# lgen-sudo/EgoM2P

Measured on NVIDIA B200. Metric: ego-b mod4 train nominal tokens/sec (whole job), higher is better.
Workload: dtype bf16

## Files before the change

egom2p_b200/csrc/attn_bwd.cu:

```cuda
#include "attn_common.cuh"

namespace egom2p {

constexpr int kBwdMathWarps = 8;
constexpr int kBwdThreads = 32 * (kBwdMathWarps + 7);
constexpr int kDrainWarp0 = kBwdMathWarps, kBwdTmaWarp = kBwdMathWarps + 4, kBwdMmaWarp = kBwdMathWarps + 5,
              kBwdMmaWarpB = kBwdMathWarps + 6;
constexpr int kBwdStages = 3;
constexpr int kBwdMetaBytes = 5 * kT * 4;
constexpr int kMaxQBlocks = 1024;

struct BwdParams {
  int B, H, Mq, Nk, S;
  RangeMeta meta;
  const float* lse2;
  const float* ndelta;
  float scale_log2;
  uint16_t* dK;
  uint16_t* dV;
  int64_t lddk, lddv;
  int tma_out;
};
struct BwdSmem {
  static constexpr int kTile = kT * 128;
  static constexpr int kK = 0, kV = kK + kTile, kQ = kV + kTile, kDO = kQ + kBwdStages * kTile,
                       kDS = kDO + kBwdStages * kTile,
                       kBox = kDS + 2 * kTile,
                       kMeta = kBox + 8 * 4096, kList = kMeta + kBwdStages * kBwdMetaBytes,
                       kBar = kList + kMaxQBlocks * 2, kTotal = kBar + 256 + 1024;
};
static_assert(BwdSmem::kTotal <= 232448, "attention backward exceeds the 227 KB shared memory of one CTA");


#ifdef EGOM2P_TRACE
__device__ long long g_trace[16 * 64];
#define TRACE(slot, idx)                                                                          \
  do {                                                                                            \
    if (blockIdx.x == 0 && blockIdx.y == 0 && blockIdx.z == gridDim.z - 1 && (idx) < 64 && (threadIdx.x & 31) == 0) \
      g_trace[(slot) * 64 + (idx)] = clock64();                                                   \
  } while (0)
#else
#define TRACE(slot, idx) do {} while (0)
#endif

__device__ __forceinline__ void tmem_st32(uint32_t taddr, const uint32_t (&r)[32]) {
  asm volatile(
      "tcgen05.st.sync.aligned.32x32b.x32.b32 [%0], "
      "{%1, %2, %3, %4, %5, %6, %7, %8, %9, %10, %11, %12, %13, %14, %15, %16, "
      "%17, %18, %19, %20, %21, %22, %23, %24, %25, %26, %27, %28, %29, %30, %31, %32};"
      ::"r"(taddr), "r"(r[0]), "r"(r[1]), "r"(r[2]), "r"(r[3]), "r"(r[4]), "r"(r[5]), "r"(r[6]), "r"(r[7]), "r"(r[8]),
        "r"(r[9]), "r"(r[10]), "r"(r[11]), "r"(r[12]), "r"(r[13]), "r"(r[14]), "r"(r[15]), "r"(r[16]), "r"(r[17]),
        "r"(r[18]), "r"(r[19]), "r"(r[20]), "r"(r[21]), "r"(r[22]), "r"(r[23]), "r"(r[24]), "r"(r[25]), "r"(r[26]),
        "r"(r[27]), "r"(r[28]), "r"(r[29]), "r"(r[30]), "r"(r[31])
      : "memory");
}
__device__ __forceinline__ void tmem_st16(uint32_t taddr, const uint32_t (&r)[16]) {
  asm volatile(
      "tcgen05.st.sync.aligned.32x32b.x16.b32 [%0], "
      "{%1, %2, %3, %4, %5, %6, %7, %8, %9, %10, %11, %12, %13, %14, %15, %16};"
      ::"r"(taddr), "r"(r[0]), "r"(r[1]), "r"(r[2]), "r"(r[3]), "r"(r[4]), "r"(r[5]), "r"(r[6]), "r"(r[7]), "r"(r[8]),
        "r"(r[9]), "r"(r[10]), "r"(r[11]), "r"(r[12]), "r"(r[13]), "r"(r[14]), "r"(r[15])
      : "memory");
}
__device__ __forceinline__ void tmem_st_wait() { asm volatile("tcgen05.wait::st.sync.aligned;" ::: "memory"); }
__device__ __forceinline__ float4 lds_f4(const void* p) {
  float4 v;
  asm volatile("ld.shared.v4.f32 {%0, %1, %2, %3}, [%4];" : "=f"(v.x), "=f"(v.y), "=f"(v.z), "=f"(v.w) : "r"(smem_u32(p)));
  return v;
}

__global__ void __launch_bounds__(kBwdThreads, 1)
attn_bwd_kernel(const __grid_constant__ CUtensorMap tmQ, const __grid_constant__ CUtensorMap tmDO,
                const __grid_constant__ CUtensorMap tmK, const __grid_constant__ CUtensorMap tmV,
                const __grid_constant__ CUtensorMap tmDQ, const __grid_constant__ CUtensorMap tmDK,
                const __grid_constant__ CUtensorMap tmDV, const BwdParams p) {
  extern __shared__ uint8_t smem_raw[];
  uint8_t* smem = reinterpret_cast<uint8_t*>((reinterpret_cast<uintptr_t>(smem_raw) + 1023) & ~(uintptr_t)1023);
  uint8_t *sK = smem + BwdSmem::kK, *sV = smem + BwdSmem::kV, *sQ = smem + BwdSmem::kQ, *sDO = smem + BwdSmem::kDO,
          *sDS = smem + BwdSmem::kDS, *sBox = smem + BwdSmem::kBox, *sMeta = smem + BwdSmem::kMeta;
  uint16_t* s_list = reinterpret_cast<uint16_t*>(smem + BwdSmem::kList);
  uint64_t* bars = reinterpret_cast<uint64_t*>(smem + BwdSmem::kBar);
  uint64_t* kv_full = bars;
  uint64_t* q_full = bars + 1;
  uint64_t* q_empty = q_full + kBwdStages;
  uint64_t* s_full = q_empty + kBwdStages;
  uint64_t* s_free = s_full + 1;
  uint64_t* dp_full = s_free + 1;
  uint64_t* dp_free = dp_full + 1;
  uint64_t* p_full = dp_free + 1;
  uint64_t* p_empty = p_full + 1;
  uint64_t* ds_full = p_empty + 1;
  uint64_t* ds_empty = ds_full + 1;
  uint64_t* dq_full = ds_empty + 1;
  uint64_t* dq_free = dq_full + 1;
  uint64_t* dkv_full = dq_free + 1;
  uint64_t* kv_tmem = dkv_full + 1;
  uint32_t* tmem_slot = reinterpret_cast<uint32_t*>(kv_tmem + 1);
  int* s_n = reinterpret_cast<int*>(tmem_slot + 1);

  const int warp = threadIdx.x >> 5, lane = threadIdx.x & 31;
  const int kv0 = blockIdx.x * kT, h = blockIdx.y, b = blockIdx.z;
  const int nqb = p.S / kT;
  if (warp == 0) TRACE(5, 63);
  if (warp == kDrainWarp0 && lane == 0) {
    tma_prefetch_desc(&tmQ);
    tma_prefetch_desc(&tmDO);
    tma_prefetch_desc(&tmDQ);
    tma_prefetch_desc(&tmDK);
    tma_prefetch_desc(&tmDV);
  }
  if (warp == kBwdTmaWarp && lane == 0) {
    mbar_init(kv_full, 1);
    fence_mbar_init();
    mbar_expect_tx(kv_full, 2 * BwdSmem::kTile);
    tma_load_2d(sK, &tmK, kv_full, h * kD, b * p.Nk + kv0);
    tma_load_2d(sV, &tmV, kv_full, h * kD, b * p.Nk + kv0);
    for (int i = 0; i < kBwdStages; ++i) { mbar_init(&q_full[i], 1); mbar_init(&q_empty[i], 1); }
    mbar_init(s_full, 1);   mbar_init(s_free, kBwdMathWarps);
    mbar_init(dp_full, 1);  mbar_init(dp_free, 1);
    mbar_init(p_full, kBwdMathWarps);  mbar_init(p_empty, 1);
    mbar_init(ds_full, kBwdMathWarps); mbar_init(ds_empty, 1);
    mbar_init(dq_full, 1);  mbar_init(dq_free, 4);
    mbar_init(dkv_full, 1);
    mbar_init(kv_tmem, kBwdMathWarps);
    fence_mbar_init();
    TRACE(5, 57);
  }
  auto issue_q_block = [&](int qblk, int st) {
    const int r0 = qblk * kT;
    uint8_t* meta = sMeta + st * kBwdMetaBytes;
    const int64_t hoff = ((int64_t)b * p.H + h) * p.S + r0, roff = (int64_t)b * p.S + r0;
    mbar_expect_tx(&q_full[st], 2 * BwdSmem::kTile + kBwdMetaBytes);
    tma_load_2d(sQ + st * BwdSmem::kTile, &tmQ, &q_full[st], h * kD, b * p.Mq + r0);
    tma_load_2d(sDO + st * BwdSmem::kTile, &tmDO, &q_full[st], h * kD, b * p.Mq + r0);
    bulk_load(meta + 0 * 512, p.lse2 + hoff, 512, &q_full[st]);
    bulk_load(meta + 1 * 512, p.ndelta + hoff, 512, &q_full[st]);
    bulk_load(meta + 2 * 512, p.meta.row_lo + roff, 512, &q_full[st]);
    bulk_load(meta + 3 * 512, p.meta.row_hi + roff, 512, &q_full[st]);
    bulk_load(meta + 4 * 512, p.meta.row_scale + roff, 512, &q_full[st]);
  };
  if (warp == kBwdTmaWarp) {
    int first = -1;
    for (int i0 = 0; i0 < nqb && first < 0; i0 += 32) {
      const int i = i0 + lane;
      bool take = false;
      if (i < nqb) {
        const int64_t o = ((int64_t)b * nqb + i) * 2;
        const int lo = min(p.meta.blk_lo[o], p.meta.blk_lo[o + 1]), hi = max(p.meta.blk_hi[o], p.meta.blk_hi[o + 1]);
        take = hi > kv0 && lo < kv0 + kT;
      }
      const unsigned msk = __ballot_sync(0xffffffffu, take);
      if (msk) first = i0 + __ffs(msk) - 1;
    }
    __syncwarp();
    if (first >= 0 && lane == 0) issue_q_block(first, 0);
  }
  if (warp == 0) {
    int n = 0;
    for (int i0 = 0; i0 < nqb; i0 += 32) {
      const int i = i0 + lane;
      bool take = false, inside = false, normal = false;
      if (i < nqb) {
        const int64_t o = ((int64_t)b * nqb + i) * 2;
        const int lo = min(p.meta.blk_lo[o], p.meta.blk_lo[o + 1]), hi = max(p.meta.blk_hi[o], p.meta.blk_hi[o + 1]);
        take = hi > kv0 && lo < kv0 + kT;
        inside = max(p.meta.blk_lo_max[o], p.meta.blk_lo_max[o + 1]) <= kv0 &&
                 min(p.meta.blk_hi_min[o], p.meta.blk_hi_min[o + 1]) >= kv0 + kT;
        normal = p.meta.blk_lo_max[o] != INT_MAX && p.meta.blk_lo_max[o + 1] != INT_MAX;
      }
      const unsigned msk = __ballot_sync(0xffffffffu, take);
      const int pos = n + __popc(msk & ((1u << lane) - 1));
      if (take && pos < kMaxQBlocks) s_list[pos] = (uint16_t)(i | (inside ? 0x8000 : 0) | (normal ? 0x4000 : 0));
      n += __popc(msk);
    }
    if (lane == 0) *s_n = n < kMaxQBlocks ? n : kMaxQBlocks;
    TRACE(5, 55);
  }
  if (warp == kBwdMmaWarp) {
    tmem_alloc<512>(tmem_slot);
    TRACE(5, 54);
  }
  if (warp == 1) TRACE(5, 53);
  tc_fence_before();
  __syncthreads();
  tc_fence_after();
  const uint32_t tmem_base = *tmem_slot;
  const int n = *s_n;
  if (warp == 0) TRACE(5, 62);
  constexpr uint32_t cS = 0, cDP = 128, cDV = 256, cDK = 320, cDQ = 384, cK = 448, cV = 480;

  if (warp >= kBwdTmaWarp) {
    if (warp == kBwdTmaWarp) {
      if (n == 0) mbar_wait(kv_full, 0);
      if (n > 0) {
        for (int idx = 1; idx < n; ++idx) {
          const int st = idx % kBwdStages;
          mbar_wait(&q_empty[st], ((idx / kBwdStages) & 1) ^ 1);
          if (elect_one()) issue_q_block((int)(s_list[idx] & 0x3fff), st);
          __syncwarp();
        }
      }
    } else if (warp == kBwdMmaWarp) {
      if (n > 0) {
        constexpr uint32_t idesc_kk = umma_idesc_bf16(128, kT, 0, 0);
        constexpr uint32_t idesc_tm = umma_idesc_bf16(128, kD, 0, 1);
        constexpr uint32_t idesc_mm = umma_idesc_bf16(128, kD, 1, 1);
        const uint32_t tS = tmem_base + cS, tDP = tmem_base + cDP, tDQ = tmem_base + cDQ, tK = tmem_base + cK, tV = tmem_base + cV;
        const uint64_t dKm0 = umma_desc_mnmajor_sw128(smem_u32(sK), 8192);
        const uint64_t dDSm0 = umma_desc_mnmajor_sw128(smem_u32(sDS), BwdSmem::kTile);
        auto issue_s = [&](int st) {
          const uint64_t dQ0 = umma_desc_kmajor_sw128(smem_u32(sQ + st * BwdSmem::kTile));
          if (elect_one()) {
#pragma unroll
            for (int k = 0; k < 4; ++k) umma_bf16_ts(tS, tK + 8 * k, dQ0 + 2 * k, idesc_kk, k ? 1u : 0u);
            umma_commit(s_full);
          }
          __syncwarp();
        };
        auto issue_dp = [&](int st) {
          const uint64_t dDO0 = umma_desc_kmajor_sw128(smem_u32(sDO + st * BwdSmem::kTile));
          if (elect_one()) {
#pragma unroll
            for (int k = 0; k < 4; ++k) umma_bf16_ts(tDP, tV + 8 * k, dDO0 + 2 * k, idesc_kk, k ? 1u : 0u);
            umma_commit(dp_full);
          }
          __syncwarp();
        };
        mbar_wait(kv_tmem, 0);
        mbar_wait(&q_full[0], 0);
        tc_fence_after();
        issue_s(0);
        issue_dp(0);
        for (int idx = 0; idx < n; ++idx) {
          const int st1 = (idx + 1) % kBwdStages;
          const uint32_t par = idx & 1;
          if (idx + 1 < n) {
            mbar_wait(&q_full[st1], ((idx + 1) / kBwdStages) & 1);
            mbar_wait(s_free, par);
            mbar_wait(p_empty, par);
            tc_fence_after();
            TRACE(0, idx);
            issue_s(st1);
          }
          mbar_wait(ds_full, par);
          if (idx > 0) mbar_wait(dq_free, (idx - 1) & 1);
          tc_fence_after();
          TRACE(4, idx);
          if (elect_one()) {
#pragma unroll
            for (int k = 0; k < 8; ++k) umma_bf16_ss(tDQ, dDSm0 + 128 * k, dKm0 + 128 * k, idesc_mm, k ? 1u : 0u);
            umma_commit(dq_full);
            umma_commit(ds_empty);
          }
          __syncwarp();
          if (idx + 1 < n) {
            mbar_wait(dp_free, par);
            tc_fence_after();
            TRACE(2, idx);
            issue_dp(st1);
          }
        }
      }
    } else if (warp == kBwdMmaWarpB) {
      if (n > 0) {
        constexpr uint32_t idesc_tm = umma_idesc_bf16(128, kD, 0, 1);
        const uint32_t tS = tmem_base + cS, tDP = tmem_base + cDP, tDV = tmem_base + cDV, tDK = tmem_base + cDK;
        for (int idx = 0; idx < n; ++idx) {
          const int st = idx % kBwdStages;
          const uint32_t par = idx & 1;
          mbar_wait(p_full, par);
          tc_fence_after();
          TRACE(1, idx);
          const uint64_t dDOm0 = umma_desc_mnmajor_sw128(smem_u32(sDO + st * BwdSmem::kTile), 8192);
          if (elect_one()) {
#pragma unroll
            for (int k = 0; k < 8; ++k)
              umma_bf16_ts(tDV, tS + (k < 4 ? 8 * k : 64 + 8 * (k - 4)), dDOm0 + 128 * k, idesc_tm, (idx | k) ? 1u : 0u);
            umma_commit(p_empty);
          }
          __syncwarp();
          mbar_wait(ds_full, par);
          tc_fence_after();
          TRACE(3, idx);
          const uint64_t dQm0 = umma_desc_mnmajor_sw128(smem_u32(sQ + st * BwdSmem::kTile), 8192);
          if (elect_one()) {
#pragma unroll
            for (int k = 0; k < 8; ++k)
              umma_bf16_ts(tDK, tDP + (k < 4 ? 8 * k : 64 + 8 * (k - 4)), dQm0 + 128 * k, idesc_tm, (idx | k) ? 1u : 0u);
            umma_commit(&q_empty[st]);
            umma_commit(dp_free);
            if (idx == n - 1) umma_commit(dkv_full);
          }
          __syncwarp();
        }
      }
    }
  } else if (warp >= kDrainWarp0) {
    const int quarter = warp & 3;
    uint8_t* box0 = sBox + quarter * 8192;
    const uint32_t t_dq = tmem_base + ((uint32_t)(quarter * 32) << 16) + cDQ;
    for (int idx = 0; idx < n; ++idx) {
      const int r0 = (int)(s_list[idx] & 0x3fff) * kT + quarter * 32;
      mbar_wait(dq_full, idx & 1);
      tc_fence_after();
      if (warp == kDrainWarp0) TRACE(11, idx);
      const bool live = r0 < p.Mq;
      if (lane == 0) tma_store_wait_read();
      __syncwarp();
#pragma unroll
      for (int hb = 0; hb < 2; ++hb) {
        uint32_t v[32];
        uint8_t* box = box0 + hb * 4096;
        tmem_ld32(t_dq + hb * 32, v);
        tmem_ld_wait();
        if (hb == 1) {
          tc_fence_before();
          __syncwarp();
          if (lane == 0) mbar_arrive(dq_free);
        }
        if (live) {
#pragma unroll
          for (int j = 0; j < 8; ++j)
            *reinterpret_cast<uint4*>(box + lane * 128 + ((j ^ (lane & 7)) << 4)) = make_uint4(v[4 * j], v[4 * j + 1], v[4 * j + 2], v[4 * j + 3]);
          fence_async_smem();
          __syncwarp();
          if (lane == 0) {
            tma_reduce_add_2d(&tmDQ, box, h * kD + hb * 32, b * p.Mq + r0);
            tma_store_commit();
          }
        }
      }
      if (warp == kDrainWarp0) TRACE(12, idx);
    }
    if (lane == 0) tma_store_wait_read();
  } else {
    const int quarter = warp & 3, half = warp >> 2;
    const int trow = quarter * 32 + lane;
    const int kidx = kv0 + trow;
    const uint32_t t_lane = tmem_base + ((uint32_t)(quarter * 32) << 16);
    uint8_t* pDS = sDS + half * BwdSmem::kTile;
    const float SC = p.scale_log2, RN = p.scale_log2 * kLn2;
    if (n > 0) {
      mbar_wait(kv_full, 0);
      if (warp == 0) TRACE(5, 56);
      uint32_t kw[16], vw[16];
#pragma unroll
      for (int c = 0; c < 4; ++c) {
        const uint4 a = *reinterpret_cast<const uint4*>(sK + swz_off(trow, half * 4 + c));
        const uint4 d = *reinterpret_cast<const uint4*>(sV + swz_off(trow, half * 4 + c));
        kw[4 * c] = a.x; kw[4 * c + 1] = a.y; kw[4 * c + 2] = a.z; kw[4 * c + 3] = a.w;
        vw[4 * c] = d.x; vw[4 * c + 1] = d.y; vw[4 * c + 2] = d.z; vw[4 * c + 3] = d.w;
      }
      tmem_st16(t_lane + cK + half * 16, kw);
      tmem_st16(t_lane + cV + half * 16, vw);
      tmem_st_wait();
      tc_fence_before();
      __syncwarp();
      if (lane == 0) mbar_arrive(kv_tmem);
      if (warp == 0) TRACE(5, 58);
    }
    for (int idx = 0; idx < n; ++idx) {
      const int st = idx % kBwdStages;
      const uint32_t par = idx & 1;
      const bool inside = (s_list[idx] & 0x8000) != 0, normal = (s_list[idx] & 0x4000) != 0;
      const float* m_ls = reinterpret_cast<const float*>(sMeta + st * kBwdMetaBytes) + half * 64;
      const float* m_nd = m_ls + kT;
      const int* m_lo = reinterpret_cast<const int*>(m_ls + 2 * kT);
      const int* m_hi = m_lo + kT;
      const float* m_rs = m_ls + 4 * kT;
      uint32_t pp[32];
      {
        uint32_t s0[32], s1[32];
        if (warp == 0) TRACE(5, idx);
        mbar_wait(&q_full[st], (idx / kBwdStages) & 1);
        mbar_wait(s_full, par);
        tc_fence_after();
        if (warp == 0) TRACE(6, idx);
        tmem_ld32(t_lane + cS + half * 64, s0);
        tmem_ld32(t_lane + cS + half * 64 + 32, s1);
        tmem_ld_wait();
        tc_fence_before();
        __syncwarp();
        if (lane == 0) mbar_arrive(s_free);
        if (inside) {
#pragma unroll
          for (int c4 = 0; c4 < 8; ++c4) {
            const float4 la = lds_f4(m_ls + 4 * c4), lb = lds_f4(m_ls + 32 + 4 * c4);
            s0[4 * c4] = __float_as_uint(fmaf(__uint_as_float(s0[4 * c4]), SC, -la.x));
            s0[4 * c4 + 1] = __float_as_uint(fmaf(__uint_as_float(s0[4 * c4 + 1]), SC, -la.y));
            s0[4 * c4 + 2] = __float_as_uint(fmaf(__uint_as_float(s0[4 * c4 + 2]), SC, -la.z));
            s0[4 * c4 + 3] = __float_as_uint(fmaf(__uint_as_float(s0[4 * c4 + 3]), SC, -la.w));
            s1[4 * c4] = __float_as_uint(fmaf(__uint_as_float(s1[4 * c4]), SC, -lb.x));
            s1[4 * c4 + 1] = __float_as_uint(fmaf(__uint_as_float(s1[4 * c4 + 1]), SC, -lb.y));
            s1[4 * c4 + 2] = __float_as_uint(fmaf(__uint_as_float(s1[4 * c4 + 2]), SC, -lb.z));
            s1[4 * c4 + 3] = __float_as_uint(fmaf(__uint_as_float(s1[4 * c4 + 3]), SC, -lb.w));
          }
#pragma unroll
          for (int c = 0; c < 32; ++c) {
            s0[c] = __float_as_uint((c & 3) == 3 ? ex2_poly(__uint_as_float(s0[c])) : ex2(__uint_as_float(s0[c])));
            s1[c] = __float_as_uint((c & 3) == 3 ? ex2_poly(__uint_as_float(s1[c])) : ex2(__uint_as_float(s1[c])));
          }
#pragma unroll
          for (int c = 0; c < 16; ++c) {
            pp[c] = pack_bf16(__uint_as_float(s0[2 * c]), __uint_as_float(s0[2 * c + 1]));
            pp[16 + c] = pack_bf16(__uint_as_float(s1[2 * c]), __uint_as_float(s1[2 * c + 1]));
          }
        } else if (normal) {
#pragma unroll
          for (int c4 = 0; c4 < 8; ++c4) {
#pragma unroll
            for (int g = 0; g < 2; ++g) {
              uint32_t(&sv)[32] = g ? s1 : s0;
              const float4 l = lds_f4(m_ls + g * 32 + 4 * c4), lo = lds_f4(m_lo + g * 32 + 4 * c4), hi = lds_f4(m_hi + g * 32 + 4 * c4);
              const float lv[4] = {l.x, l.y, l.z, l.w};
              const int lov[4] = {__float_as_int(lo.x), __float_as_int(lo.y), __float_as_int(lo.z), __float_as_int(lo.w)};
              const int hiv[4] = {__float_as_int(hi.x), __float_as_int(hi.y), __float_as_int(hi.z), __float_as_int(hi.w)};
#pragma unroll
              for (int u = 0; u < 4; ++u) {
                const bool ok = kidx >= lov[u] && kidx < hiv[u];
                sv[4 * c4 + u] = ok ? __float_as_uint(fmaf(__uint_as_float(sv[4 * c4 + u]), SC, -lv[u])) : 0xff800000u;
              }
            }
          }
#pragma unroll
          for (int c = 0; c < 32; ++c) {
            s0[c] = __float_as_uint(ex2(__uint_as_float(s0[c])));
            s1[c] = __float_as_uint(ex2(__uint_as_float(s1[c])));
          }
#pragma unroll
          for (int c = 0; c < 16; ++c) {
            pp[c] = pack_bf16(__uint_as_float(s0[2 * c]), __uint_as_float(s0[2 * c + 1]));
            pp[16 + c] = pack_bf16(__uint_as_float(s1[2 * c]), __uint_as_float(s1[2 * c + 1]));
          }
        } else {
#pragma unroll
          for (int c = 0; c < 32; ++c) {
            float e[2];
#pragma unroll
            for (int u = 0; u < 2; ++u) {
              const int q = 2 * c + u;
              const float rs = m_rs[q];
              const bool ok = kidx >= m_lo[q] && kidx < m_hi[q];
              const float sv = __uint_as_float(q < 32 ? s0[q & 31] : s1[q & 31]);
              e[u] = ok ? ex2(fmaf(rs != 0.f ? sv : 0.f, rs, -m_ls[q])) : 0.f;
            }
            pp[c] = pack_bf16(e[0], e[1]);
          }
        }
      }
      if (warp == 0) TRACE(7, idx);
      tmem_st32(t_lane + cS + half * 64, pp);
      uint32_t d0[32];
      mbar_wait(dp_full, par);
      tc_fence_after();
      tmem_ld32(t_lane + cDP + half * 64, d0);
      tmem_st_wait();
      tc_fence_before();
      __syncwarp();
      if (lane == 0) mbar_arrive(p_full);
      if (warp == 0) TRACE(8, idx);
      auto dsmul = [&](const uint32_t (&d)[32], int hh) {
        if (inside || normal) {
#pragma unroll
          for (int c4 = 0; c4 < 8; ++c4) {
            const float4 nd = lds_f4(m_nd + hh * 32 + 4 * c4);
            const uint32_t t0 = pack_bf16(fmaf(__uint_as_float(d[4 * c4]), RN, nd.x), fmaf(__uint_as_float(d[4 * c4 + 1]), RN, nd.y));
            const uint32_t t1 = pack_bf16(fmaf(__uint_as_float(d[4 * c4 + 2]), RN, nd.z), fmaf(__uint_as_float(d[4 * c4 + 3]), RN, nd.w));
            asm("mul.rn.bf16x2 %0, %1, %2;" : "=r"(pp[hh * 16 + 2 * c4]) : "r"(pp[hh * 16 + 2 * c4]), "r"(t0));
            asm("mul.rn.bf16x2 %0, %1, %2;" : "=r"(pp[hh * 16 + 2 * c4 + 1]) : "r"(pp[hh * 16 + 2 * c4 + 1]), "r"(t1));
          }
        } else {
#pragma unroll
          for (int c4 = 0; c4 < 8; ++c4) {
            const float4 nd = lds_f4(m_nd + hh * 32 + 4 * c4);
            const float4 rs = lds_f4(m_rs + hh * 32 + 4 * c4);
            const uint32_t t0 = pack_bf16(fmaf(__uint_as_float(d[4 * c4]), rs.x * kLn2, nd.x), fmaf(__uint_as_float(d[4 * c4 + 1]), rs.y * kLn2, nd.y));
            const uint32_t t1 = pack_bf16(fmaf(__uint_as_float(d[4 * c4 + 2]), rs.z * kLn2, nd.z), fmaf(__uint_as_float(d[4 * c4 + 3]), rs.w * kLn2, nd.w));
            asm("mul.rn.bf16x2 %0, %1, %2;" : "=r"(pp[hh * 16 + 2 * c4]) : "r"(pp[hh * 16 + 2 * c4]), "r"(t0));
            asm("mul.rn.bf16x2 %0, %1, %2;" : "=r"(pp[hh * 16 + 2 * c4 + 1]) : "r"(pp[hh * 16 + 2 * c4 + 1]), "r"(t1));
          }
        }
      };
      tmem_ld_wait();
      if (warp == 0) TRACE(9, idx);
      dsmul(d0, 0);
      if (warp == 0) TRACE(13, idx);
      tmem_ld32(t_lane + cDP + half * 64 + 32, d0);
      if (idx > 0) mbar_wait(ds_empty, (idx - 1) & 1);
      tmem_ld_wait();
      if (warp == 0) TRACE(14, idx);
      dsmul(d0, 1);
      if (warp == 0) TRACE(15, idx);
      tmem_st32(t_lane + cDP + half * 64, pp);
#pragma unroll
      for (int c8 = 0; c8 < 8; ++c8)
        *reinterpret_cast<uint4*>(pDS + swz_off(trow, c8)) = make_uint4(pp[4 * c8], pp[4 * c8 + 1], pp[4 * c8 + 2], pp[4 * c8 + 3]);
      fence_async_smem();
      tmem_st_wait();
      tc_fence_before();
      __syncwarp();
      if (lane == 0) mbar_arrive(ds_full);
      if (warp == 0) TRACE(10, idx);
    }
    if (n > 0) {
      mbar_wait(dkv_full, 0);
      tc_fence_after();
    }
    if (warp == 0) TRACE(5, 61);
#pragma unroll 1
    for (int which = 0; which < 2; ++which) {
      uint32_t v[32];
      if (n > 0) {
        tmem_ld32(t_lane + (which == 0 ? cDV : cDK) + half * 32, v);
        tmem_ld_wait();
      } else {
#pragma unroll
        for (int c = 0; c < 32; ++c) v[c] = 0u;
      }
      uint4 pk[4];
#pragma unroll
      for (int c8 = 0; c8 < 4; ++c8) {
        pk[c8].x = pack_bf16(__uint_as_float(v[c8 * 8 + 0]), __uint_as_float(v[c8 * 8 + 1]));
        pk[c8].y = pack_bf16(__uint_as_float(v[c8 * 8 + 2]), __uint_as_float(v[c8 * 8 + 3]));
        pk[c8].z = pack_bf16(__uint_as_float(v[c8 * 8 + 4]), __uint_as_float(v[c8 * 8 + 5]));
        pk[c8].w = pack_bf16(__uint_as_float(v[c8 * 8 + 6]), __uint_as_float(v[c8 * 8 + 7]));
      }
      if (p.tma_out) {
        uint8_t* stage = which == 0 ? sQ : sDO;
#pragma unroll
        for (int c8 = 0; c8 < 4; ++c8) *reinterpret_cast<uint4*>(stage + swz_off(trow, half * 4 + c8)) = pk[c8];
        if (warp == 0) TRACE(5, 52 - which);
      } else if (kidx < p.Nk) {
        uint16_t* out = (which == 0 ? p.dV + ((int64_t)b * p.Nk + kidx) * p.lddv : p.dK + ((int64_t)b * p.Nk + kidx) * p.lddk) +
                        h * kD + half * 32;
#pragma unroll
        for (int c8 = 0; c8 < 4; ++c8) reinterpret_cast<uint4*>(out)[c8] = pk[c8];
      }
    }
    if (p.tma_out) {
      fence_async_smem();
      asm volatile("bar.sync 1, 256;" ::: "memory");
      if (warp == 0) TRACE(5, 50);
      if (warp == 0 && lane == 0) {
        tma_store_2d(&tmDV, sQ, h * kD, b * p.Nk + kv0);
        tma_store_2d(&tmDK, sDO, h * kD, b * p.Nk + kv0);
        tma_store_commit();
        tma_store_wait_read();
      }
    }
    if (warp == 0) TRACE(5, 60);
  }
  tc_fence_before();
  __syncthreads();
  if (warp == 0) TRACE(5, 59);
  if (warp == kBwdMmaWarp) {
    tc_fence_after();
    tmem_dealloc<512>(tmem_base);
  }
}

__global__ void __launch_bounds__(256) attn_bwd_prep_kernel(const uint16_t* __restrict__ O, const uint16_t* __restrict__ dO,
                                                            int64_t ldo, const float* __restrict__ row_scale, int B, int H,
                                                            int Mq, int S, float* __restrict__ ndelta, float* __restrict__ dq_acc) {
  const int64_t wid = (int64_t)blockIdx.x * 8 + (threadIdx.x >> 5);
  const int lane = threadIdx.x & 31;
  if (wid >= (int64_t)B * S) return;
  const int b = (int)(wid / S), r = (int)(wid % S);
  if (r >= Mq) {
    for (int hh = lane; hh < H; hh += 32) ndelta[((int64_t)b * H + hh) * S + r] = 0.f;
    return;
  }
  const float rs = row_scale[wid] * kLn2;
  const uint16_t* po = O + ((int64_t)b * Mq + r) * ldo;
  const uint16_t* pd = dO + ((int64_t)b * Mq + r) * ldo;
  float4* acc = reinterpret_cast<float4*>(dq_acc + ((int64_t)b * Mq + r) * (int64_t)H * kD);
  const int chunks = H * 8;
  for (int c0 = 0; c0 < chunks; c0 += 32) {
    const int c = c0 + lane;
    float part = 0.f;
    if (c < chunks) {
      const uint4 a = reinterpret_cast<const uint4*>(po)[c], g = reinterpret_cast<const uint4*>(pd)[c];
      const uint32_t aw[4] = {a.x, a.y, a.z, a.w}, gw[4] = {g.x, g.y, g.z, g.w};
#pragma unroll
      for (int u = 0; u < 4; ++u) {
        const float2 fa = __bfloat1622float2(*reinterpret_cast<const __nv_bfloat162*>(&aw[u]));
        const float2 fg = __bfloat1622float2(*reinterpret_cast<const __nv_bfloat162*>(&gw[u]));
        part += fa.x * fg.x + fa.y * fg.y;
      }
      acc[2 * c] = make_float4(0.f, 0.f, 0.f, 0.f);
      acc[2 * c + 1] = make_float4(0.f, 0.f, 0.f, 0.f);
    }
    part += __shfl_xor_sync(0xffffffffu, part, 1);
    part += __shfl_xor_sync(0xffffffffu, part, 2);
    part += __shfl_xor_sync(0xffffffffu, part, 4);
    if (c < chunks && (lane & 7) == 0) ndelta[((int64_t)b * H + (c >> 3)) * S + r] = -part * rs;
  }
}

__global__ void __launch_bounds__(256) attn_bwd_dq_cast_kernel(const float* __restrict__ acc, int64_t rows, int cols8,
                                                               uint16_t* __restrict__ dq, int64_t lddq) {
  const int64_t total = rows * cols8;
  for (int64_t i = (int64_t)blockIdx.x * blockDim.x + threadIdx.x; i < total; i += (int64_t)gridDim.x * blockDim.x) {
    const int64_t r = i / cols8;
    const int c = (int)(i % cols8);
    const float4 a = reinterpret_cast<const float4*>(acc + r * cols8 * 8)[2 * c];
    const float4 g = reinterpret_cast<const float4*>(acc + r * cols8 * 8)[2 * c + 1];
    uint4 pk;
    pk.x = pack_bf16(a.x, a.y); pk.y = pack_bf16(a.z, a.w); pk.z = pack_bf16(g.x, g.y); pk.w = pack_bf16(g.z, g.w);
    reinterpret_cast<uint4*>(dq + r * lddq)[c] = pk;
  }
}

}

#ifdef EGOM2P_TRACE
extern "C" int egom2p_debug_attn_trace(long long* host_dst) {
  return (int)cudaMemcpyFromSymbol(host_dst, egom2p::g_trace, sizeof(egom2p::g_trace));
}
#endif

extern "C" int64_t egom2p_attn_bwd_scratch_bytes(int32_t B, int32_t H, int32_t Mq) {
  using namespace egom2p;
  return align256((int64_t)B * H * padS(Mq) * 4) + align256((int64_t)B * Mq * H * kD * 4) + 256;
}

extern "C" int egom2p_attn_bwd(const uint16_t* Q, const uint16_t* K, const uint16_t* V, const uint16_t* O, const uint16_t* dO,
                               const float* lse, int32_t B, int32_t H, int32_t Mq, int32_t Nk, int64_t ldq, int64_t ldk,
                               int64_t ldv, int64_t ldo, const void* meta, float scale, void* scratch, uint16_t* dQ,
                               uint16_t* dK, uint16_t* dV, int64_t lddq, int64_t lddk, int64_t lddv, void* stream_) {
  using namespace egom2p;
  cudaStream_t stream = (cudaStream_t)stream_;
  EGO_REQUIRE(Q && O && dO && lse && meta && scratch && dQ && B > 0 && H > 0 && Mq > 0 && Nk >= 0, "attn_bwd: bad argument");
  EGO_REQUIRE(((uintptr_t)scratch & 255) == 0 && ((uintptr_t)lse & 255) == 0 && ((uintptr_t)meta & 255) == 0,
              "attn_bwd: scratch / lse / meta must be 256-byte aligned");
  EGO_REQUIRE(lddq % 8 == 0 && ((uintptr_t)dQ & 15) == 0 && ldo % 8 == 0 && ((uintptr_t)O & 15) == 0 && ((uintptr_t)dO & 15) == 0,
              "attn_bwd: dQ / O / dO alignment");
  const int S = padS(Mq);
  EGO_REQUIRE(S / kT <= kMaxQBlocks, "attn_bwd: Mq too large (max %d)", kMaxQBlocks * kT);
  RangeMeta rm = carve_meta(const_cast<void*>(meta), B, Mq);
  float* ndelta = reinterpret_cast<float*>(scratch);
  float* dq_acc = reinterpret_cast<float*>(reinterpret_cast<char*>(scratch) + align256((int64_t)B * H * S * 4));

  attn_bwd_prep_kernel<<<(unsigned)(((int64_t)B * S + 7) / 8), 256, 0, stream>>>(O, dO, ldo, rm.row_scale, B, H, Mq, S, ndelta, dq_acc);
  int rc = check_launch("attn_bwd prep");
  if (rc) return rc;
  if (Nk > 0) {
    EGO_REQUIRE(K && V && dK && dV, "attn_bwd: K / V / dK / dV missing");
    EGO_REQUIRE(lddk % 8 == 0 && lddv % 8 == 0 && ((uintptr_t)dK & 15) == 0 && ((uintptr_t)dV & 15) == 0, "attn_bwd: dK/dV alignment");
    static std::atomic<uint64_t> attr_done{0};
    if ((rc = ensure_dyn_smem(attn_bwd_kernel, BwdSmem::kTotal, attr_done, "attn_bwd"))) return rc;
    CUtensorMap tmQ, tmDO, tmK, tmV, tmDQ, tmDK, tmDV;
    if ((rc = make_tmap_bf16_2d(&tmQ, Q, (uint64_t)B * Mq, (uint64_t)H * kD, ldq, kT, kD))) return rc;
    if ((rc = make_tmap_bf16_2d(&tmDO, dO, (uint64_t)B * Mq, (uint64_t)H * kD, ldo, kT, kD))) return rc;
    if ((rc = make_tmap_bf16_2d(&tmK, K, (uint64_t)B * Nk, (uint64_t)H * kD, ldk, kT, kD))) return rc;
    if ((rc = make_tmap_bf16_2d(&tmV, V, (uint64_t)B * Nk, (uint64_t)H * kD, ldv, kT, kD))) return rc;
    if ((rc = make_tmap_2d(&tmDQ, dq_acc, 4, (uint64_t)B * Mq, (uint64_t)H * kD, (uint64_t)H * kD, 32, 32))) return rc;
    const int tma_out = (Nk % kT == 0 || B == 1) ? 1 : 0;
    if (tma_out) {
      if ((rc = make_tmap_bf16_2d(&tmDK, dK, (uint64_t)B * Nk, (uint64_t)H * kD, lddk, kT, kD))) return rc;
      if ((rc = make_tmap_bf16_2d(&tmDV, dV, (uint64_t)B * Nk, (uint64_t)H * kD, lddv, kT, kD))) return rc;
    } else {
      tmDK = tmK;
      tmDV = tmV;
    }
    BwdParams pb{B, H, Mq, Nk, S, rm, lse, ndelta, scale * kLog2e, dK, dV, lddk, lddv, tma_out};
    attn_bwd_kernel<<<dim3((Nk + kT - 1) / kT, H, B), kBwdThreads, BwdSmem::kTotal, stream>>>(tmQ, tmDO, tmK, tmV, tmDQ, tmDK, tmDV, pb);
    if ((rc = check_launch("attn_bwd"))) return rc;
  }
  const int64_t rows = (int64_t)B * Mq;
  const int cols8 = H * kD / 8;
  const int64_t total = rows * cols8;
  attn_bwd_dq_cast_kernel<<<(unsigned)((total + 255) / 256 < 148 * 16 ? (total + 255) / 256 : 148 * 16), 256, 0, stream>>>(dq_acc, rows, cols8, dQ, lddq);
  return check_launch("attn_bwd dq cast");
}
```

egom2p_b200/csrc/common.cuh:

```cuda
#pragma once
#include <cuda.h>
#include <cuda_bf16.h>
#include <cuda_runtime.h>
#include <stdint.h>
#include <atomic>
#include <cstdio>

#include "../../include/egom2p_b200.h"

namespace egom2p {

void set_error(const char* fmt, ...);
int check_launch(const char* what);
#define EGO_REQUIRE(cond, ...)                 \
  do {                                         \
    if (!(cond)) {                             \
      ::egom2p::set_error(__VA_ARGS__);        \
      return EGOM2P_ERR_INVALID;               \
    }                                          \
  } while (0)

int make_tmap_bf16_2d(CUtensorMap* out, const void* base, uint64_t rows, uint64_t cols, uint64_t ld,
                      uint32_t box_rows, uint32_t box_cols);

int make_tmap_2d(CUtensorMap* out, const void* base, int elem_bytes, uint64_t rows, uint64_t cols, uint64_t ld,
                 uint32_t box_rows, uint32_t box_cols);

template <typename Kern>
static inline int ensure_dyn_smem(Kern kern, int bytes, std::atomic<uint64_t>& done, const char* what) {
  int dev = 0;
  cudaGetDevice(&dev);
  const uint64_t bit = 1ull << (dev & 63);
  if (done.load(std::memory_order_acquire) & bit) return 0;
  cudaError_t e = cudaFuncSetAttribute(kern, cudaFuncAttributeMaxDynamicSharedMemorySize, bytes);
  if (e != cudaSuccess) {
    set_error("%s: cudaFuncSetAttribute(%d B smem): %s", what, bytes, cudaGetErrorString(e));
    return EGOM2P_ERR_CUDA;
  }
  done.fetch_or(bit, std::memory_order_release);
  return 0;
}
static inline int device_sm_count() {
  static std::atomic<int> cached[64];
  int dev = 0;
  cudaGetDevice(&dev);
  int v = cached[dev & 63].load(std::memory_order_relaxed);
  if (v <= 0) {
    cudaDeviceGetAttribute(&v, cudaDevAttrMultiProcessorCount, dev);
    if (v <= 0) v = 148;
    cached[dev & 63].store(v, std::memory_order_relaxed);
  }
  return v;
}

#ifdef __CUDACC__

__device__ __forceinline__ uint32_t smem_u32(const void* p) {
  return static_cast<uint32_t>(__cvta_generic_to_shared(p));
}
__device__ __forceinline__ bool elect_one() {
  uint32_t pred;
  asm volatile(
      "{\n\t.reg .pred p;\n\telect.sync _|p, 0xffffffff;\n\tselp.b32 %0, 1, 0, p;\n\t}\n"
      : "=r"(pred));
  return pred != 0;
}

__device__ __forceinline__ void mbar_init(uint64_t* bar, uint32_t count) {
  asm volatile("mbarrier.init.shared::cta.b64 [%0], %1;" ::"r"(smem_u32(bar)), "r"(count));
}
__device__ __forceinline__ void fence_mbar_init() {
  asm volatile("fence.mbarrier_init.release.cluster;" ::: "memory");
}
__device__ __forceinline__ void mbar_expect_tx(uint64_t* bar, uint32_t bytes) {
  asm volatile("mbarrier.arrive.expect_tx.shared::cta.b64 _, [%0], %1;" ::"r"(smem_u32(bar)), "r"(bytes)
               : "memory");
}
__device__ __forceinline__ void mbar_arrive(uint64_t* bar) {
  asm volatile("mbarrier.arrive.shared::cta.b64 _, [%0];" ::"r"(smem_u32(bar)) : "memory");
}
__device__ __forceinline__ bool mbar_try_wait(uint64_t* bar, uint32_t parity) {
  uint32_t ok;
  asm volatile(
      "{\n\t.reg .pred p;\n\t"
      "mbarrier.try_wait.parity.shared::cta.b64 p, [%1], %2, %3;\n\t"
      "selp.b32 %0, 1, 0, p;\n\t}\n"
      : "=r"(ok)
      : "r"(smem_u32(bar)), "r"(parity), "r"(1000000u)
      : "memory");
  return ok != 0;
}
static __device__ __noinline__ void mbar_wait_slow(uint64_t* bar, uint32_t parity) {
  for (uint32_t spins = 0; !mbar_try_wait(bar, parity); ++spins) {
    if (spins > 20000u) {
      printf("egom2p: mbarrier timeout block (%d,%d,%d) thread %d\n", blockIdx.x, blockIdx.y, blockIdx.z, threadIdx.x);
      __trap();
    }
  }
}
__device__ __forceinline__ void mbar_wait(uint64_t* bar, uint32_t parity) {
  if (!mbar_try_wait(bar, parity)) mbar_wait_slow(bar, parity);
}

__device__ __forceinline__ void fence_async_smem() {
  asm volatile("fence.proxy.async.shared::cta;" ::: "memory");
}
__device__ __forceinline__ void tc_fence_before() { asm volatile("tcgen05.fence::before_thread_sync;" ::: "memory"); }
__device__ __forceinline__ void tc_fence_after() { asm volatile("tcgen05.fence::after_thread_sync;" ::: "memory"); }

__device__ __forceinline__ void tma_prefetch_desc(const CUtensorMap* m) {
  asm volatile("prefetch.tensormap [%0];" ::"l"(reinterpret_cast<uint64_t>(m)) : "memory");
}
__device__ __forceinline__ void tma_load_2d(void* smem_dst, const CUtensorMap* m, uint64_t* bar, int crd0, int crd1) {
  asm volatile(
      "cp.async.bulk.tensor.2d.shared::cluster.global.mbarrier::complete_tx::bytes [%0], [%1, {%3, %4}], [%2];"
      ::"r"(smem_u32(smem_dst)), "l"(reinterpret_cast<uint64_t>(m)), "r"(smem_u32(bar)), "r"(crd0), "r"(crd1)
      : "memory");
}

__device__ __forceinline__ void tma_load_2d_pair(void* smem_dst, const CUtensorMap* m, uint64_t* bar, int crd0, int crd1) {
  asm volatile(
      "cp.async.bulk.tensor.2d.cta_group::2.shared::cluster.global.mbarrier::complete_tx::bytes [%0], [%1, {%3, %4}], [%2];"
      ::"r"(smem_u32(smem_dst)), "l"(reinterpret_cast<uint64_t>(m)), "r"(smem_u32(bar) & 0xFEFFFFFFu), "r"(crd0), "r"(crd1)
      : "memory");
}
__device__ __forceinline__ uint32_t cluster_map(const void* p, uint32_t rank) {
  uint32_t r;
  asm volatile("mapa.shared::cluster.u32 %0, %1, %2;" : "=r"(r) : "r"(smem_u32(p)), "r"(rank));
  return r;
}
__device__ __forceinline__ void mbar_arrive_cluster(uint32_t cluster_addr) {
  asm volatile("mbarrier.arrive.shared::cluster.b64 _, [%0];" ::"r"(cluster_addr) : "memory");
}
__device__ __forceinline__ void mbar_expect_tx_cluster(uint32_t cluster_addr, uint32_t bytes) {
  asm volatile("mbarrier.arrive.expect_tx.shared::cluster.b64 _, [%0], %1;" ::"r"(cluster_addr), "r"(bytes) : "memory");
}
__device__ __forceinline__ void clc_try_cancel_multicast(void* resp16, uint64_t* bar) {
  asm volatile(
      "clusterlaunchcontrol.try_cancel.async.shared::cta.mbarrier::complete_tx::bytes.multicast::cluster::all.b128 [%0], [%1];"
      ::"r"(smem_u32(resp16)), "r"(smem_u32(bar)) : "memory");
}
__device__ __forceinline__ bool clc_decode(const void* resp16, int& first_ctaid_x) {
  uint32_t valid, x;
  asm volatile(
      "{\n\t.reg .pred p1;\n\t.reg .b128 r;\n\t"
      "ld.shared.b128 r, [%2];\n\t"
      "clusterlaunchcontrol.query_cancel.is_canceled.pred.b128 p1, r;\n\t"
      "selp.u32 %1, 1, 0, p1;\n\t"
      "mov.u32 %0, 0;\n\t"
      "@p1 clusterlaunchcontrol.query_cancel.get_first_ctaid.v4.b32.b128 {%0, _, _, _}, r;\n\t}\n"
      : "=r"(x), "=r"(valid) : "r"(smem_u32(resp16)) : "memory");
  first_ctaid_x = (int)x;
  return valid != 0;
}
__device__ __forceinline__ uint32_t cluster_ctarank() {
  uint32_t r;
  asm volatile("mov.u32 %0, %%cluster_ctarank;" : "=r"(r));
  return r;
}
__device__ __forceinline__ void cluster_sync() {
  asm volatile("barrier.cluster.arrive.release.aligned;\n\tbarrier.cluster.wait.acquire.aligned;" ::: "memory");
}

__device__ __forceinline__ void tma_store_2d(const CUtensorMap* m, const void* smem_src, int crd0, int crd1) {
  asm volatile("cp.async.bulk.tensor.2d.global.shared::cta.bulk_group [%0, {%2, %3}], [%1];"
               ::"l"(reinterpret_cast<uint64_t>(m)), "r"(smem_u32(smem_src)), "r"(crd0), "r"(crd1)
               : "memory");
}
__device__ __forceinline__ void tma_reduce_add_2d(const CUtensorMap* m, const void* smem_src, int crd0, int crd1) {
  asm volatile("cp.reduce.async.bulk.tensor.2d.global.shared::cta.add.tile.bulk_group [%0, {%2, %3}], [%1];"
               ::"l"(reinterpret_cast<uint64_t>(m)), "r"(smem_u32(smem_src)), "r"(crd0), "r"(crd1)
               : "memory");
}
__device__ __forceinline__ void tma_store_commit() { asm volatile("cp.async.bulk.commit_group;" ::: "memory"); }
__device__ __forceinline__ void tma_store_wait_read() { asm volatile("cp.async.bulk.wait_group.read 0;" ::: "memory"); }
__device__ __forceinline__ void tma_store_wait_read1() { asm volatile("cp.async.bulk.wait_group.read 1;" ::: "memory"); }
__device__ __forceinline__ void tma_store_wait_all() { asm volatile("cp.async.bulk.wait_group 0;" ::: "memory"); }

template <int kCols>
__device__ __forceinline__ void tmem_alloc(uint32_t* smem_out) {
  asm volatile("tcgen05.alloc.cta_group::1.sync.aligned.shared::cta.b32 [%0], %1;" ::"r"(smem_u32(smem_out)), "n"(kCols)
               : "memory");
  asm volatile("tcgen05.relinquish_alloc_permit.cta_group::1.sync.aligned;" ::: "memory");
}
template <int kCols>
__device__ __forceinline__ void tmem_dealloc(uint32_t taddr) {
  asm volatile("tcgen05.dealloc.cta_group::1.sync.aligned.b32 %0, %1;" ::"r"(taddr), "n"(kCols) : "memory");
}

__device__ __forceinline__ uint64_t umma_desc_kmajor_sw128(uint32_t saddr) {
  uint64_t d = 0;
  d |= (uint64_t)((saddr & 0x3FFFF) >> 4);
  d |= (uint64_t)1 << 16;
  d |= (uint64_t)(1024 >> 4) << 32;
  d |= (uint64_t)1 << 46;
  d |= (uint64_t)2 << 61;
  return d;
}
__device__ __forceinline__ uint64_t umma_desc_mnmajor_sw128(uint32_t saddr, uint32_t lbo_bytes) {
  uint64_t d = 0;
  d |= (uint64_t)((saddr & 0x3FFFF) >> 4);
  d |= (uint64_t)((lbo_bytes >> 4) & 0x3FFF) << 16;
  d |= (uint64_t)(1024 >> 4) << 32;
  d |= (uint64_t)1 << 46;
  d |= (uint64_t)2 << 61;
  return d;
}
__host__ __device__ constexpr uint32_t umma_idesc_bf16(int M, int N, int a_mn, int b_mn) {
  return (1u << 4) | (1u << 7) | (1u << 10) | ((uint32_t)a_mn << 15) | ((uint32_t)b_mn << 16) |
         ((uint32_t)(N >> 3) << 17) | ((uint32_t)(M >> 4) << 24);
}
__device__ __forceinline__ void umma_bf16_ss(uint32_t tmem_d, uint64_t desc_a, uint64_t desc_b, uint32_t idesc,
                                             uint32_t accumulate) {
  asm volatile(
      "{\n\t.reg .pred p;\n\tsetp.ne.b32 p, %4, 0;\n\t"
      "tcgen05.mma.cta_group::1.kind::f16 [%0], %1, %2, %3, p;\n\t}\n"
      ::"r"(tmem_d), "l"(desc_a), "l"(desc_b), "r"(idesc), "r"(accumulate)
      : "memory");
}
__device__ __forceinline__ void umma_commit(uint64_t* bar) {
  asm volatile("tcgen05.commit.cta_group::1.mbarrier::arrive::one.shared::cluster.b64 [%0];" ::"r"(smem_u32(bar))
               : "memory");
}
__device__ __forceinline__ void umma_bf16_ss_pair(uint32_t tmem_d, uint64_t desc_a, uint64_t desc_b, uint32_t idesc, uint32_t accumulate) {
  asm volatile(
      "{\n\t.reg .pred p;\n\tsetp.ne.b32 p, %4, 0;\n\t"
      "tcgen05.mma.cta_group::2.kind::f16 [%0], %1, %2, %3, p;\n\t}\n"
      ::"r"(tmem_d), "l"(desc_a), "l"(desc_b), "r"(idesc), "r"(accumulate)
      : "memory");
}
__device__ __forceinline__ void umma_commit_pair(uint64_t* bar) {
  asm volatile("tcgen05.commit.cta_group::2.mbarrier::arrive::one.shared::cluster.multicast::cluster.b64 [%0], %1;"
               ::"r"(smem_u32(bar)), "h"((uint16_t)3) : "memory");
}
template <int kCols>
__device__ __forceinline__ void tmem_alloc_pair(uint32_t* smem_out) {
  asm volatile("tcgen05.alloc.cta_group::2.sync.aligned.shared::cta.b32 [%0], %1;" ::"r"(smem_u32(smem_out)), "n"(kCols) : "memory");
  asm volatile("tcgen05.relinquish_alloc_permit.cta_group::2.sync.aligned;" ::: "memory");
}
template <int kCols>
__device__ __forceinline__ void tmem_dealloc_pair(uint32_t taddr) {
  asm volatile("tcgen05.dealloc.cta_group::2.sync.aligned.b32 %0, %1;" ::"r"(taddr), "n"(kCols) : "memory");
}
__device__ __forceinline__ void tmem_ld32(uint32_t taddr, uint32_t (&r)[32]) {
  asm volatile(
      "tcgen05.ld.sync.aligned.32x32b.x32.b32 "
      "{%0, %1, %2, %3, %4, %5, %6, %7, %8, %9, %10, %11, %12, %13, %14, %15, "
      "%16, %17, %18, %19, %20, %21, %22, %23, %24, %25, %26, %27, %28, %29, %30, %31}, [%32];"
      : "=r"(r[0]), "=r"(r[1]), "=r"(r[2]), "=r"(r[3]), "=r"(r[4]), "=r"(r[5]), "=r"(r[6]), "=r"(r[7]), "=r"(r[8]),
        "=r"(r[9]), "=r"(r[10]), "=r"(r[11]), "=r"(r[12]), "=r"(r[13]), "=r"(r[14]), "=r"(r[15]), "=r"(r[16]),
        "=r"(r[17]), "=r"(r[18]), "=r"(r[19]), "=r"(r[20]), "=r"(r[21]), "=r"(r[22]), "=r"(r[23]), "=r"(r[24]),
        "=r"(r[25]), "=r"(r[26]), "=r"(r[27]), "=r"(r[28]), "=r"(r[29]), "=r"(r[30]), "=r"(r[31])
      : "r"(taddr)
      : "memory");
}
__device__ __forceinline__ void tmem_ld_wait() { asm volatile("tcgen05.wait::ld.sync.aligned;" ::: "memory"); }

__device__ __forceinline__ float warp_sum(float v) {
#pragma unroll
  for (int o = 16; o > 0; o >>= 1) v += __shfl_xor_sync(0xffffffffu, v, o);
  return v;
}
__device__ __forceinline__ float warp_max(float v) {
#pragma unroll
  for (int o = 16; o > 0; o >>= 1) v = fmaxf(v, __shfl_xor_sync(0xffffffffu, v, o));
  return v;
}
__device__ __forceinline__ uint32_t pack_bf16(float a, float b) {
  __nv_bfloat162 t = __floats2bfloat162_rn(a, b);
  return *reinterpret_cast<uint32_t*>(&t);
}
#endif

}
```

Before: 712,500.

## Make attention backward persistent via cluster launch control with overlapped KV tiles

Turns the attention backward kernel into a persistent-style kernel. The TMA warp uses cluster launch control try_cancel to claim further (kv-block, head, batch) tiles and publishes each tile through a double-buffered tile descriptor with full/empty barriers. K is double-buffered and the next tile's S/dP MMAs are issued before the current tile finishes, so per-CTA launch, TMEM allocation and pipeline ramp costs are amortised and tail gaps are hidden. dK/dV output is staged in smaller 32-row boxes. This adds considerable barrier and phase-tracking complexity, with a risk of deadlock or ordering bugs.

```diff
diff --git a/egom2p_b200/csrc/attn_bwd.cu b/egom2p_b200/csrc/attn_bwd.cu
--- a/egom2p_b200/csrc/attn_bwd.cu
+++ b/egom2p_b200/csrc/attn_bwd.cu
@@ -6,6 +6,7 @@
 constexpr int kBwdThreads = 32 * (kBwdMathWarps + 7);
 constexpr int kDrainWarp0 = kBwdMathWarps, kBwdTmaWarp = kBwdMathWarps + 4, kBwdMmaWarp = kBwdMathWarps + 5,
               kBwdMmaWarpB = kBwdMathWarps + 6;
+constexpr int kBwdTileReaders = kBwdMathWarps + 4 + 2;
 constexpr int kBwdStages = 3;
 constexpr int kBwdMetaBytes = 5 * kT * 4;
 constexpr int kMaxQBlocks = 1024;
@@ -21,26 +22,43 @@
   int64_t lddk, lddv;
   int tma_out;
 };
+struct BwdTile {
+  int n, kv0, h, b;
+};
 struct BwdSmem {
   static constexpr int kTile = kT * 128;
-  static constexpr int kK = 0, kV = kK + kTile, kQ = kV + kTile, kDO = kQ + kBwdStages * kTile,
+  static constexpr int kK = 0,
+                       kV = kK + 2 * kTile, kQ = kV + kTile, kDO = kQ + kBwdStages * kTile,
                        kDS = kDO + kBwdStages * kTile,
                        kBox = kDS + 2 * kTile,
                        kMeta = kBox + 8 * 4096, kList = kMeta + kBwdStages * kBwdMetaBytes,
-                       kBar = kList + kMaxQBlocks * 2, kTotal = kBar + 256 + 1024;
+                       kCtl = kList + 2 * kMaxQBlocks * 2,
+                       kTotal = kCtl + 512 + 1024;
 };
 static_assert(BwdSmem::kTotal <= 232448, "attention backward exceeds the 227 KB shared memory of one CTA");
 
 
 #ifdef EGOM2P_TRACE
 __device__ long long g_trace[16 * 64];
-#define TRACE(slot, idx)                                                                          \
-  do {                                                                                            \
-    if (blockIdx.x == 0 && blockIdx.y == 0 && blockIdx.z == gridDim.z - 1 && (idx) < 64 && (threadIdx.x & 31) == 0) \
-      g_trace[(slot) * 64 + (idx)] = clock64();                                                   \
+__device__ long long g_trace_tile[64 * 4];
+__device__ long long g_trace_cta[4];
+#define TRACE_ON (blockIdx.x == 0 && blockIdx.y == 0 && blockIdx.z == gridDim.z - 1 && (threadIdx.x & 31) == 0)
+#define TRACE(slot, idx)                                              \
+  do {                                                                \
+    if (TRACE_ON && (idx) < 64) g_trace[(slot) * 64 + (idx)] = clock64(); \
+  } while (0)
+#define TRACE_TILE(t, field, value)                                     \
+  do {                                                                  \
+    if (TRACE_ON && (t) < 64) g_trace_tile[(t) * 4 + (field)] = (value); \
+  } while (0)
+#define TRACE_CTA(i)                          \
+  do {                                        \
+    if (TRACE_ON) g_trace_cta[i] = clock64(); \
   } while (0)
 #else
 #define TRACE(slot, idx) do {} while (0)
+#define TRACE_TILE(t, field, value) do {} while (0)
+#define TRACE_CTA(i) do {} while (0)
 #endif
 
 __device__ __forceinline__ void tmem_st32(uint32_t taddr, const uint32_t (&r)[32]) {
@@ -79,9 +97,13 @@
   uint8_t *sK = smem + BwdSmem::kK, *sV = smem + BwdSmem::kV, *sQ = smem + BwdSmem::kQ, *sDO = smem + BwdSmem::kDO,
           *sDS = smem + BwdSmem::kDS, *sBox = smem + BwdSmem::kBox, *sMeta = smem + BwdSmem::kMeta;
   uint16_t* s_list = reinterpret_cast<uint16_t*>(smem + BwdSmem::kList);
-  uint64_t* bars = reinterpret_cast<uint64_t*>(smem + BwdSmem::kBar);
+  uint4* clc_resp = reinterpret_cast<uint4*>(smem + BwdSmem::kCtl);
+  BwdTile* s_tile = reinterpret_cast<BwdTile*>(clc_resp + 1);
+  uint64_t* bars = reinterpret_cast<uint64_t*>(s_tile + 2);
   uint64_t* kv_full = bars;
-  uint64_t* q_full = bars + 1;
+  uint64_t* k_empty = kv_full + 2;
+  uint64_t* v_free = k_empty + 2;
+  uint64_t* q_full = v_free + 1;
   uint64_t* q_empty = q_full + kBwdStages;
   uint64_t* s_full = q_empty + kBwdStages;
   uint64_t* s_free = s_full + 1;
@@ -94,183 +116,236 @@
   uint64_t* dq_full = ds_empty + 1;
   uint64_t* dq_free = dq_full + 1;
   uint64_t* dkv_full = dq_free + 1;
-  uint64_t* kv_tmem = dkv_full + 1;
-  uint32_t* tmem_slot = reinterpret_cast<uint32_t*>(kv_tmem + 1);
-  int* s_n = reinterpret_cast<int*>(tmem_slot + 1);
+  uint64_t* dkv_drained = dkv_full + 1;
+  uint64_t* kv_tmem = dkv_drained + 1;
+  uint64_t* tile_full = kv_tmem + 1;
+  uint64_t* tile_empty = tile_full + 2;
+  uint64_t* clc_full = tile_empty + 2;
+  uint32_t* tmem_slot = reinterpret_cast<uint32_t*>(clc_full + 1);
 
   const int warp = threadIdx.x >> 5, lane = threadIdx.x & 31;
-  const int kv0 = blockIdx.x * kT, h = blockIdx.y, b = blockIdx.z;
   const int nqb = p.S / kT;
-  if (warp == 0) TRACE(5, 63);
+  if (warp == 0) TRACE_CTA(0);
   if (warp == kDrainWarp0 && lane == 0) {
     tma_prefetch_desc(&tmQ);
     tma_prefetch_desc(&tmDO);
+    tma_prefetch_desc(&tmK);
+    tma_prefetch_desc(&tmV);
     tma_prefetch_desc(&tmDQ);
     tma_prefetch_desc(&tmDK);
     tma_prefetch_desc(&tmDV);
   }
   if (warp == kBwdTmaWarp && lane == 0) {
-    mbar_init(kv_full, 1);
-    fence_mbar_init();
-    mbar_expect_tx(kv_full, 2 * BwdSmem::kTile);
-    tma_load_2d(sK, &tmK, kv_full, h * kD, b * p.Nk + kv0);
-    tma_load_2d(sV, &tmV, kv_full, h * kD, b * p.Nk + kv0);
+    for (int i = 0; i < 2; ++i) {
+      mbar_init(&kv_full[i], 1);   mbar_init(&k_empty[i], 1);
+      mbar_init(&tile_full[i], 1); mbar_init(&tile_empty[i], kBwdTileReaders);
+    }
+    mbar_init(v_free, kBwdMathWarps);
     for (int i = 0; i < kBwdStages; ++i) { mbar_init(&q_full[i], 1); mbar_init(&q_empty[i], 1); }
     mbar_init(s_full, 1);   mbar_init(s_free, kBwdMathWarps);
     mbar_init(dp_full, 1);  mbar_init(dp_free, 1);
     mbar_init(p_full, kBwdMathWarps);  mbar_init(p_empty, 1);
     mbar_init(ds_full, kBwdMathWarps); mbar_init(ds_empty, 1);
     mbar_init(dq_full, 1);  mbar_init(dq_free, 4);
-    mbar_init(dkv_full, 1);
+    mbar_init(dkv_full, 1); mbar_init(dkv_drained, 4);
     mbar_init(kv_tmem, kBwdMathWarps);
+    mbar_init(clc_full, 1);
     fence_mbar_init();
-    TRACE(5, 57);
   }
-  auto issue_q_block = [&](int qblk, int st) {
-    const int r0 = qblk * kT;
-    uint8_t* meta = sMeta + st * kBwdMetaBytes;
-    const int64_t hoff = ((int64_t)b * p.H + h) * p.S + r0, roff = (int64_t)b * p.S + r0;
-    mbar_expect_tx(&q_full[st], 2 * BwdSmem::kTile + kBwdMetaBytes);
-    tma_load_2d(sQ + st * BwdSmem::kTile, &tmQ, &q_full[st], h * kD, b * p.Mq + r0);
-    tma_load_2d(sDO + st * BwdSmem::kTile, &tmDO, &q_full[st], h * kD, b * p.Mq + r0);
-    bulk_load(meta + 0 * 512, p.lse2 + hoff, 512, &q_full[st]);
-    bulk_load(meta + 1 * 512, p.ndelta + hoff, 512, &q_full[st]);
-    bulk_load(meta + 2 * 512, p.meta.row_lo + roff, 512, &q_full[st]);
-    bulk_load(meta + 3 * 512, p.meta.row_hi + roff, 512, &q_full[st]);
-    bulk_load(meta + 4 * 512, p.meta.row_scale + roff, 512, &q_full[st]);
-  };
-  if (warp == kBwdTmaWarp) {
-    int first = -1;
-    for (int i0 = 0; i0 < nqb && first < 0; i0 += 32) {
-      const int i = i0 + lane;
-      bool take = false;
-      if (i < nqb) {
-        const int64_t o = ((int64_t)b * nqb + i) * 2;
-        const int lo = min(p.meta.blk_lo[o], p.meta.blk_lo[o + 1]), hi = max(p.meta.blk_hi[o], p.meta.blk_hi[o + 1]);
-        take = hi > kv0 && lo < kv0 + kT;
-      }
-      const unsigned msk = __ballot_sync(0xffffffffu, take);
-      if (msk) first = i0 + __ffs(msk) - 1;
-    }
-    __syncwarp();
-    if (first >= 0 && lane == 0) issue_q_block(first, 0);
-  }
-  if (warp == 0) {
-    int n = 0;
-    for (int i0 = 0; i0 < nqb; i0 += 32) {
-      const int i = i0 + lane;
-      bool take = false, inside = false, normal = false;
-      if (i < nqb) {
-        const int64_t o = ((int64_t)b * nqb + i) * 2;
-        const int lo = min(p.meta.blk_lo[o], p.meta.blk_lo[o + 1]), hi = max(p.meta.blk_hi[o], p.meta.blk_hi[o + 1]);
-        take = hi > kv0 && lo < kv0 + kT;
-        inside = max(p.meta.blk_lo_max[o], p.meta.blk_lo_max[o + 1]) <= kv0 &&
-                 min(p.meta.blk_hi_min[o], p.meta.blk_hi_min[o + 1]) >= kv0 + kT;
-        normal = p.meta.blk_lo_max[o] != INT_MAX && p.meta.blk_lo_max[o + 1] != INT_MAX;
-      }
-      const unsigned msk = __ballot_sync(0xffffffffu, take);
-      const int pos = n + __popc(msk & ((1u << lane) - 1));
-      if (take && pos < kMaxQBlocks) s_list[pos] = (uint16_t)(i | (inside ? 0x8000 : 0) | (normal ? 0x4000 : 0));
-      n += __popc(msk);
-    }
-    if (lane == 0) *s_n = n < kMaxQBlocks ? n : kMaxQBlocks;
-    TRACE(5, 55);
-  }
-  if (warp == kBwdMmaWarp) {
-    tmem_alloc<512>(tmem_slot);
-    TRACE(5, 54);
-  }
-  if (warp == 1) TRACE(5, 53);
+  if (warp == kBwdMmaWarp) tmem_alloc<512>(tmem_slot);
   tc_fence_before();
   __syncthreads();
   tc_fence_after();
   const uint32_t tmem_base = *tmem_slot;
-  const int n = *s_n;
-  if (warp == 0) TRACE(5, 62);
+  if (warp == 0) TRACE_CTA(1);
   constexpr uint32_t cS = 0, cDP = 128, cDV = 256, cDK = 320, cDQ = 384, cK = 448, cV = 480;
+
+  auto wait_tile = [&](int t) -> BwdTile {
+    mbar_wait(&tile_full[t & 1], (t >> 1) & 1);
+    return s_tile[t & 1];
+  };
+  auto release_tile = [&](int t) {
+    __syncwarp();
+    if (lane == 0) mbar_arrive(&tile_empty[t & 1]);
+  };
 
   if (warp >= kBwdTmaWarp) {
     if (warp == kBwdTmaWarp) {
-      if (n == 0) mbar_wait(kv_full, 0);
-      if (n > 0) {
-        for (int idx = 1; idx < n; ++idx) {
-          const int st = idx % kBwdStages;
-          mbar_wait(&q_empty[st], ((idx / kBwdStages) & 1) ^ 1);
-          if (elect_one()) issue_q_block((int)(s_list[idx] & 0x3fff), st);
+      int x = blockIdx.x, hh = blockIdx.y, bb = blockIdx.z;
+      bool more = true;
+      int g = 0, lt = 0;
+      for (int t = 0;; ++t) {
+        const int slot = t & 1;
+        uint16_t* list = s_list + slot * kMaxQBlocks;
+        const int kv0 = x * kT;
+        mbar_wait(&tile_empty[slot], ((t >> 1) & 1) ^ 1);
+        int n = -1;
+        if (more) {
+          if (elect_one()) {
+            mbar_expect_tx(clc_full, 16);
+            clc_try_cancel(clc_resp, clc_full);
+          }
           __syncwarp();
-        }
+          n = 0;
+          for (int i0 = 0; i0 < nqb; i0 += 32) {
+            const int i = i0 + lane;
+            bool take = false, inside = false, normal = false;
+            if (i < nqb) {
+              const int64_t o = ((int64_t)bb * nqb + i) * 2;
+              const int lo = min(p.meta.blk_lo[o], p.meta.blk_lo[o + 1]), hi = max(p.meta.blk_hi[o], p.meta.blk_hi[o + 1]);
+              take = hi > kv0 && lo < kv0 + kT;
+              inside = max(p.meta.blk_lo_max[o], p.meta.blk_lo_max[o + 1]) <= kv0 &&
+                       min(p.meta.blk_hi_min[o], p.meta.blk_hi_min[o + 1]) >= kv0 + kT;
+              normal = p.meta.blk_lo_max[o] != INT_MAX && p.meta.blk_lo_max[o + 1] != INT_MAX;
+            }
+            const unsigned msk = __ballot_sync(0xffffffffu, take);
+            const int pos = n + __popc(msk & ((1u << lane) - 1));
+            if (take && pos < kMaxQBlocks) list[pos] = (uint16_t)(i | (inside ? 0x8000 : 0) | (normal ? 0x4000 : 0));
+            n += __popc(msk);
+          }
+          n = min(n, kMaxQBlocks);
+        }
+        if (lane == 0) s_tile[slot] = BwdTile{n, kv0, hh, bb};
+        __threadfence_block();
+        __syncwarp();
+        if (lane == 0) mbar_arrive(&tile_full[slot]);
+        TRACE_TILE(t, 0, g);
+        TRACE_TILE(t, 1, n);
+        if (n < 0) break;
+        if (n > 0) {
+          const int kb = lt & 1;
+          mbar_wait(&k_empty[kb], ((lt >> 1) & 1) ^ 1);
+          mbar_wait(v_free, (lt & 1) ^ 1);
+          if (elect_one()) {
+            mbar_expect_tx(&kv_full[kb], 2 * BwdSmem::kTile);
+            tma_load_2d(sK + kb * BwdSmem::kTile, &tmK, &kv_full[kb], hh * kD, bb * p.Nk + kv0);
+            tma_load_2d(sV, &tmV, &kv_full[kb], hh * kD, bb * p.Nk + kv0);
+          }
+          __syncwarp();
+          for (int idx = 0; idx < n; ++idx, ++g) {
+            const int st = g % kBwdStages;
+            const int r0 = (int)(list[idx] & 0x3fff) * kT;
+            mbar_wait(&q_empty[st], ((g / kBwdStages) & 1) ^ 1);
+            if (elect_one()) {
+              uint8_t* meta = sMeta + st * kBwdMetaBytes;
+              const int64_t hoff = ((int64_t)bb * p.H + hh) * p.S + r0, roff = (int64_t)bb * p.S + r0;
+              mbar_expect_tx(&q_full[st], 2 * BwdSmem::kTile + kBwdMetaBytes);
+              tma_load_2d(sQ + st * BwdSmem::kTile, &tmQ, &q_full[st], hh * kD, bb * p.Mq + r0);
+              tma_load_2d(sDO + st * BwdSmem::kTile, &tmDO, &q_full[st], hh * kD, bb * p.Mq + r0);
+              bulk_load(meta + 0 * 512, p.lse2 + hoff, 512, &q_full[st]);
+              bulk_load(meta + 1 * 512, p.ndelta + hoff, 512, &q_full[st]);
+              bulk_load(meta + 2 * 512, p.meta.row_lo + roff, 512, &q_full[st]);
+              bulk_load(meta + 3 * 512, p.meta.row_hi + roff, 512, &q_full[st]);
+              bulk_load(meta + 4 * 512, p.meta.row_scale + roff, 512, &q_full[st]);
+            }
+            __syncwarp();
+          }
+          ++lt;
+        }
+        mbar_wait(clc_full, t & 1);
+        more = clc_decode_xyz(clc_resp, x, hh, bb);
+        fence_async_smem();
+        __syncwarp();
       }
     } else if (warp == kBwdMmaWarp) {
-      if (n > 0) {
-        constexpr uint32_t idesc_kk = umma_idesc_bf16(128, kT, 0, 0);
-        constexpr uint32_t idesc_tm = umma_idesc_bf16(128, kD, 0, 1);
-        constexpr uint32_t idesc_mm = umma_idesc_bf16(128, kD, 1, 1);
-        const uint32_t tS = tmem_base + cS, tDP = tmem_base + cDP, tDQ = tmem_base + cDQ, tK = tmem_base + cK, tV = tmem_base + cV;
-        const uint64_t dKm0 = umma_desc_mnmajor_sw128(smem_u32(sK), 8192);
-        const uint64_t dDSm0 = umma_desc_mnmajor_sw128(smem_u32(sDS), BwdSmem::kTile);
-        auto issue_s = [&](int st) {
-          const uint64_t dQ0 = umma_desc_kmajor_sw128(smem_u32(sQ + st * BwdSmem::kTile));
-          if (elect_one()) {
-#pragma unroll
-            for (int k = 0; k < 4; ++k) umma_bf16_ts(tS, tK + 8 * k, dQ0 + 2 * k, idesc_kk, k ? 1u : 0u);
-            umma_commit(s_full);
-          }
-          __syncwarp();
-        };
-        auto issue_dp = [&](int st) {
-          const uint64_t dDO0 = umma_desc_kmajor_sw128(smem_u32(sDO + st * BwdSmem::kTile));
-          if (elect_one()) {
-#pragma unroll
-            for (int k = 0; k < 4; ++k) umma_bf16_ts(tDP, tV + 8 * k, dDO0 + 2 * k, idesc_kk, k ? 1u : 0u);
-            umma_commit(dp_full);
-          }
-          __syncwarp();
-        };
-        mbar_wait(kv_tmem, 0);
-        mbar_wait(&q_full[0], 0);
-        tc_fence_after();
-        issue_s(0);
-        issue_dp(0);
-        for (int idx = 0; idx < n; ++idx) {
-          const int st1 = (idx + 1) % kBwdStages;
-          const uint32_t par = idx & 1;
-          if (idx + 1 < n) {
-            mbar_wait(&q_full[st1], ((idx + 1) / kBwdStages) & 1);
+      constexpr uint32_t idesc_kk = umma_idesc_bf16(128, kT, 0, 0);
+      constexpr uint32_t idesc_mm = umma_idesc_bf16(128, kD, 1, 1);
+      const uint32_t tS = tmem_base + cS, tDP = tmem_base + cDP, tDQ = tmem_base + cDQ, tK = tmem_base + cK, tV = tmem_base + cV;
+      const uint64_t dDSm0 = umma_desc_mnmajor_sw128(smem_u32(sDS), BwdSmem::kTile);
+      auto issue_s = [&](int st) {
+        const uint64_t dQ0 = umma_desc_kmajor_sw128(smem_u32(sQ + st * BwdSmem::kTile));
+        if (elect_one()) {
+#pragma unroll
+          for (int k = 0; k < 4; ++k) umma_bf16_ts(tS, tK + 8 * k, dQ0 + 2 * k, idesc_kk, k ? 1u : 0u);
+          umma_commit(s_full);
+        }
+        __syncwarp();
+      };
+      auto issue_dp = [&](int st) {
+        const uint64_t dDO0 = umma_desc_kmajor_sw128(smem_u32(sDO + st * BwdSmem::kTile));
+        if (elect_one()) {
+#pragma unroll
+          for (int k = 0; k < 4; ++k) umma_bf16_ts(tDP, tV + 8 * k, dDO0 + 2 * k, idesc_kk, k ? 1u : 0u);
+          umma_commit(dp_full);
+        }
+        __syncwarp();
+      };
+      int g = 0, lt = 0;
+      bool ahead = false;
+      for (int t = 0;; ++t) {
+        const int n = wait_tile(t).n;
+        if (n < 0) break;
+        release_tile(t);
+        if (n == 0) continue;
+        const uint64_t dKm0 = umma_desc_mnmajor_sw128(smem_u32(sK + (lt & 1) * BwdSmem::kTile), 8192);
+        if (!ahead) {
+          const int st = g % kBwdStages;
+          mbar_wait(kv_tmem, lt & 1);
+          mbar_wait(&q_full[st], (g / kBwdStages) & 1);
+          if (g > 0) {
+            mbar_wait(s_free, (g - 1) & 1);
+            mbar_wait(p_empty, (g - 1) & 1);
+          }
+          tc_fence_after();
+          issue_s(st);
+          if (g > 0) {
+            mbar_wait(dp_free, (g - 1) & 1);
+            tc_fence_after();
+          }
+          issue_dp(st);
+        }
+        for (int idx = 0; idx < n; ++idx, ++g) {
+          const int st1 = (g + 1) % kBwdStages;
+          const uint32_t par = g & 1;
+          ahead = idx + 1 < n;
+          if (!ahead) {
+            ahead = wait_tile(t + 1).n > 0;
+            if (ahead) mbar_wait(kv_tmem, (lt + 1) & 1);
+          }
+          if (ahead) {
+            mbar_wait(&q_full[st1], ((g + 1) / kBwdStages) & 1);
             mbar_wait(s_free, par);
             mbar_wait(p_empty, par);
             tc_fence_after();
-            TRACE(0, idx);
+            TRACE(0, g);
             issue_s(st1);
           }
           mbar_wait(ds_full, par);
-          if (idx > 0) mbar_wait(dq_free, (idx - 1) & 1);
+          if (g > 0) mbar_wait(dq_free, (g - 1) & 1);
           tc_fence_after();
-          TRACE(4, idx);
+          TRACE(4, g);
           if (elect_one()) {
 #pragma unroll
             for (int k = 0; k < 8; ++k) umma_bf16_ss(tDQ, dDSm0 + 128 * k, dKm0 + 128 * k, idesc_mm, k ? 1u : 0u);
             umma_commit(dq_full);
             umma_commit(ds_empty);
+            if (idx == n - 1) umma_commit(&k_empty[lt & 1]);
           }
           __syncwarp();
-          if (idx + 1 < n) {
+          if (ahead) {
             mbar_wait(dp_free, par);
             tc_fence_after();
-            TRACE(2, idx);
+            TRACE(2, g);
             issue_dp(st1);
           }
         }
+        ++lt;
       }
     } else if (warp == kBwdMmaWarpB) {
-      if (n > 0) {
-        constexpr uint32_t idesc_tm = umma_idesc_bf16(128, kD, 0, 1);
-        const uint32_t tS = tmem_base + cS, tDP = tmem_base + cDP, tDV = tmem_base + cDV, tDK = tmem_base + cDK;
-        for (int idx = 0; idx < n; ++idx) {
-          const int st = idx % kBwdStages;
-          const uint32_t par = idx & 1;
+      constexpr uint32_t idesc_tm = umma_idesc_bf16(128, kD, 0, 1);
+      const uint32_t tS = tmem_base + cS, tDP = tmem_base + cDP, tDV = tmem_base + cDV, tDK = tmem_base + cDK;
+      int g = 0, lt = 0;
+      for (int t = 0;; ++t) {
+        const int n = wait_tile(t).n;
+        if (n < 0) break;
+        release_tile(t);
+        for (int idx = 0; idx < n; ++idx, ++g) {
+          const int st = g % kBwdStages;
+          const uint32_t par = g & 1;
           mbar_wait(p_full, par);
+          if (idx == 0) mbar_wait(dkv_drained, (lt & 1) ^ 1);
           tc_fence_after();
-          TRACE(1, idx);
+          TRACE(1, g);
           const uint64_t dDOm0 = umma_desc_mnmajor_sw128(smem_u32(sDO + st * BwdSmem::kTile), 8192);
           if (elect_one()) {
 #pragma unroll
@@ -281,7 +356,7 @@
           __syncwarp();
           mbar_wait(ds_full, par);
           tc_fence_after();
-          TRACE(3, idx);
+          TRACE(3, g);
           const uint64_t dQm0 = umma_desc_mnmajor_sw128(smem_u32(sQ + st * BwdSmem::kTile), 8192);
           if (elect_one()) {
 #pragma unroll
@@ -293,266 +368,306 @@
           }
           __syncwarp();
         }
+        if (n > 0) ++lt;
       }
     }
   } else if (warp >= kDrainWarp0) {
     const int quarter = warp & 3;
     uint8_t* box0 = sBox + quarter * 8192;
-    const uint32_t t_dq = tmem_base + ((uint32_t)(quarter * 32) << 16) + cDQ;
-    for (int idx = 0; idx < n; ++idx) {
-      const int r0 = (int)(s_list[idx] & 0x3fff) * kT + quarter * 32;
-      mbar_wait(dq_full, idx & 1);
-      tc_fence_after();
-      if (warp == kDrainWarp0) TRACE(11, idx);
-      const bool live = r0 < p.Mq;
+    const uint32_t t_q = tmem_base + ((uint32_t)(quarter * 32) << 16);
+    int g = 0, lt = 0;
+    for (int t = 0;; ++t) {
+      const BwdTile tile = wait_tile(t);
+      if (tile.n < 0) break;
+      const uint16_t* list = s_list + (t & 1) * kMaxQBlocks;
+      auto drain_dq = [&](int idx) {
+        const int r0 = (int)(list[idx] & 0x3fff) * kT + quarter * 32;
+        mbar_wait(dq_full, g & 1);
+        tc_fence_after();
+        if (warp == kDrainWarp0) TRACE(11, g);
+        const bool live = r0 < p.Mq;
+        if (lane == 0) tma_store_wait_read();
+        __syncwarp();
+#pragma unroll
+        for (int hb = 0; hb < 2; ++hb) {
+          uint32_t v[32];
+          uint8_t* box = box0 + hb * 4096;
+          tmem_ld32(t_q + cDQ + hb * 32, v);
+          tmem_ld_wait();
+          if (hb == 1) {
+            tc_fence_before();
+            __syncwarp();
+            if (lane == 0) mbar_arrive(dq_free);
+          }
+          if (live) {
+#pragma unroll
+            for (int j = 0; j < 8; ++j)
+              *reinterpret_cast<uint4*>(box + lane * 128 + ((j ^ (lane & 7)) << 4)) = make_uint4(v[4 * j], v[4 * j + 1], v[4 * j + 2], v[4 * j + 3]);
+            fence_async_smem();
+            __syncwarp();
+            if (lane == 0) {
+              tma_reduce_add_2d(&tmDQ, box, tile.h * kD + hb * 32, tile.b * p.Mq + r0);
+              tma_store_commit();
+            }
+          }
+        }
+        if (warp == kDrainWarp0) TRACE(12, g);
+      };
+      for (int idx = 0; idx + 1 < tile.n; ++idx, ++g) drain_dq(idx);
+      const int krow = tile.kv0 + quarter * 32;
+      if (tile.n > 0) {
+        mbar_wait(dkv_full, lt & 1);
+        tc_fence_after();
+      }
       if (lane == 0) tma_store_wait_read();
       __syncwarp();
 #pragma unroll
-      for (int hb = 0; hb < 2; ++hb) {
+      for (int w = 0; w < 4; ++w) {
         uint32_t v[32];
-        uint8_t* box = box0 + hb * 4096;
-        tmem_ld32(t_dq + hb * 32, v);
-        tmem_ld_wait();
-        if (hb == 1) {
-          tc_fence_before();
-          __syncwarp();
-          if (lane == 0) mbar_arrive(dq_free);
-        }
-        if (live) {
-#pragma unroll
-          for (int j = 0; j < 8; ++j)
-            *reinterpret_cast<uint4*>(box + lane * 128 + ((j ^ (lane & 7)) << 4)) = make_uint4(v[4 * j], v[4 * j + 1], v[4 * j + 2], v[4 * j + 3]);
-          fence_async_smem();
-          __syncwarp();
-          if (lane == 0) {
-            tma_reduce_add_2d(&tmDQ, box, h * kD + hb * 32, b * p.Mq + r0);
-            tma_store_commit();
-          }
-        }
-      }
-      if (warp == kDrainWarp0) TRACE(12, idx);
+        if (tile.n > 0) {
+          tmem_ld32(t_q + ((w >> 1) == 0 ? cDV : cDK) + (w & 1) * 32, v);
+          tmem_ld_wait();
+          if (w == 3) {
+            tc_fence_before();
+            __syncwarp();
+            if (lane == 0) mbar_arrive(dkv_drained);
+          }
+        } else {
+#pragma unroll
+          for (int c = 0; c < 32; ++c) v[c] = 0u;
+        }
+        uint4 pk[4];
+#pragma unroll
+        for (int c8 = 0; c8 < 4; ++c8)
+          pk[c8] = make_uint4(pack_bf16(__uint_as_float(v[8 * c8]), __uint_as_float(v[8 * c8 + 1])),
+                              pack_bf16(__uint_as_float(v[8 * c8 + 2]), __uint_as_float(v[8 * c8 + 3])),
+                              pack_bf16(__uint_as_float(v[8 * c8 + 4]), __uint_as_float(v[8 * c8 + 5])),
+                              pack_bf16(__uint_as_float(v[8 * c8 + 6]), __uint_as_float(v[8 * c8 + 7])));
+        if (p.tma_out) {
+#pragma unroll
+          for (int c8 = 0; c8 < 4; ++c8)
+            *reinterpret_cast<uint4*>(box0 + (w >> 1) * 4096 + lane * 128 + ((((w & 1) * 4 + c8) ^ (lane & 7)) << 4)) = pk[c8];
+        } else if (krow + lane < p.Nk) {
+          const int64_t row = (int64_t)tile.b * p.Nk + krow + lane;
+          uint16_t* out = ((w >> 1) == 0 ? p.dV + row * p.lddv : p.dK + row * p.lddk) + tile.h * kD + (w & 1) * 32;
+#pragma unroll
+          for (int c8 = 0; c8 < 4; ++c8) reinterpret_cast<uint4*>(out)[c8] = pk[c8];
+        }
+      }
+      if (p.tma_out) {
+        fence_async_smem();
+        __syncwarp();
+        if (lane == 0) {
+          tma_store_2d(&tmDV, box0, tile.h * kD, tile.b * p.Nk + krow);
+          tma_store_2d(&tmDK, box0 + 4096, tile.h * kD, tile.b * p.Nk + krow);
+          tma_store_commit();
+        }
+      }
+      if (tile.n > 0) {
+        ++lt;
+        drain_dq(tile.n - 1);
+        ++g;
+      }
+      release_tile(t);
+      if (warp == kDrainWarp0) TRACE_TILE(t, 3, clock64());
     }
     if (lane == 0) tma_store_wait_read();
   } else {
     const int quarter = warp & 3, half = warp >> 2;
     const int trow = quarter * 32 + lane;
-    const int kidx = kv0 + trow;
     const uint32_t t_lane = tmem_base + ((uint32_t)(quarter * 32) << 16);
-    uint8_t* pDS = sDS + half * BwdSmem::kTile;
+    const uint32_t aDS = smem_u32(sDS + half * BwdSmem::kTile);
     const float SC = p.scale_log2, RN = p.scale_log2 * kLn2;
-    if (n > 0) {
-      mbar_wait(kv_full, 0);
-      if (warp == 0) TRACE(5, 56);
-      uint32_t kw[16], vw[16];
-#pragma unroll
-      for (int c = 0; c < 4; ++c) {
-        const uint4 a = *reinterpret_cast<const uint4*>(sK + swz_off(trow, half * 4 + c));
-        const uint4 d = *reinterpret_cast<const uint4*>(sV + swz_off(trow, half * 4 + c));
-        kw[4 * c] = a.x; kw[4 * c + 1] = a.y; kw[4 * c + 2] = a.z; kw[4 * c + 3] = a.w;
-        vw[4 * c] = d.x; vw[4 * c + 1] = d.y; vw[4 * c + 2] = d.z; vw[4 * c + 3] = d.w;
-      }
-      tmem_st16(t_lane + cK + half * 16, kw);
-      tmem_st16(t_lane + cV + half * 16, vw);
+    auto copy_kv = [&](int l) {
+      mbar_wait(&kv_full[l & 1], (l >> 1) & 1);
+      const uint8_t* k = sK + (l & 1) * BwdSmem::kTile;
+#pragma unroll
+      for (int m = 0; m < 2; ++m) {
+        uint32_t w[16];
+#pragma unroll
+        for (int c = 0; c < 4; ++c) {
+          const uint4 a = *reinterpret_cast<const uint4*>((m ? sV : k) + swz_off(trow, half * 4 + c));
+          w[4 * c] = a.x; w[4 * c + 1] = a.y; w[4 * c + 2] = a.z; w[4 * c + 3] = a.w;
+        }
+        tmem_st16(t_lane + (m ? cV : cK) + half * 16, w);
+      }
       tmem_st_wait();
       tc_fence_before();
       __syncwarp();
-      if (lane == 0) mbar_arrive(kv_tmem);
-      if (warp == 0) TRACE(5, 58);
-    }
-    for (int idx = 0; idx < n; ++idx) {
-      const int st = idx % kBwdStages;
-      const uint32_t par = idx & 1;
-      const bool inside = (s_list[idx] & 0x8000) != 0, normal = (s_list[idx] & 0x4000) != 0;
-      const float* m_ls = reinterpret_cast<const float*>(sMeta + st * kBwdMetaBytes) + half * 64;
-      const float* m_nd = m_ls + kT;
-      const int* m_lo = reinterpret_cast<const int*>(m_ls + 2 * kT);
-      const int* m_hi = m_lo + kT;
-      const float* m_rs = m_ls + 4 * kT;
-      uint32_t pp[32];
-      {
-        uint32_t s0[32], s1[32];
-        if (warp == 0) TRACE(5, idx);
-        mbar_wait(&q_full[st], (idx / kBwdStages) & 1);
-        mbar_wait(s_full, par);
+      if (lane == 0) {
+        mbar_arrive(v_free);
+        mbar_arrive(kv_tmem);
+      }
+    };
+    int g = 0, cur = 0;
+    auto copy_next_kv = [&]() {
+      copy_kv((cur >> 1) & 3);
+      cur = (cur & ~6) | ((cur + 2) & 6);
+    };
+    for (;; cur += 8) {
+      const int t = cur >> 3;
+      const BwdTile tile = wait_tile(t);
+      if (tile.n < 0) break;
+      const int gend = g + tile.n;
+      const uint16_t* list = s_list + (t & 1) * kMaxQBlocks - g;
+      const int kidx = tile.kv0 + trow;
+      if (warp == 0) TRACE_TILE(t, 2, clock64());
+      if (tile.n > 0 && !(cur & 1)) copy_next_kv();
+      cur &= ~1;
+      for (; g < gend; ++g) {
+        const int st = g % kBwdStages;
+        const uint32_t par = g & 1;
+        const bool inside = (list[g] & 0x8000) != 0, normal = (list[g] & 0x4000) != 0;
+        const float* m_ls = reinterpret_cast<const float*>(sMeta + st * kBwdMetaBytes) + half * 64;
+        const float* m_nd = m_ls + kT;
+        const int* m_lo = reinterpret_cast<const int*>(m_ls + 2 * kT);
+        const int* m_hi = m_lo + kT;
+        const float* m_rs = m_ls + 4 * kT;
+        uint32_t pp[32];
+        {
+          uint32_t s0[32], s1[32];
+          if (warp == 0) TRACE(5, g);
+          mbar_wait(&q_full[st], (g / kBwdStages) & 1);
+          mbar_wait(s_full, par);
+          tc_fence_after();
+          if (warp == 0) TRACE(6, g);
+          tmem_ld32(t_lane + cS + half * 64, s0);
+          tmem_ld32(t_lane + cS + half * 64 + 32, s1);
+          tmem_ld_wait();
+          tc_fence_before();
+          __syncwarp();
+          if (lane == 0) mbar_arrive(s_free);
+          if (inside) {
+#pragma unroll
+            for (int c4 = 0; c4 < 8; ++c4) {
+              const float4 la = lds_f4(m_ls + 4 * c4), lb = lds_f4(m_ls + 32 + 4 * c4);
+              s0[4 * c4] = __float_as_uint(fmaf(__uint_as_float(s0[4 * c4]), SC, -la.x));
+              s0[4 * c4 + 1] = __float_as_uint(fmaf(__uint_as_float(s0[4 * c4 + 1]), SC, -la.y));
+              s0[4 * c4 + 2] = __float_as_uint(fmaf(__uint_as_float(s0[4 * c4 + 2]), SC, -la.z));
+              s0[4 * c4 + 3] = __float_as_uint(fmaf(__uint_as_float(s0[4 * c4 + 3]), SC, -la.w));
+              s1[4 * c4] = __float_as_uint(fmaf(__uint_as_float(s1[4 * c4]), SC, -lb.x));
+              s1[4 * c4 + 1] = __float_as_uint(fmaf(__uint_as_float(s1[4 * c4 + 1]), SC, -lb.y));
+              s1[4 * c4 + 2] = __float_as_uint(fmaf(__uint_as_float(s1[4 * c4 + 2]), SC, -lb.z));
+              s1[4 * c4 + 3] = __float_as_uint(fmaf(__uint_as_float(s1[4 * c4 + 3]), SC, -lb.w));
+            }
+#pragma unroll
+            for (int c = 0; c < 32; ++c) {
+              s0[c] = __float_as_uint((c & 3) == 3 ? ex2_poly(__uint_as_float(s0[c])) : ex2(__uint_as_float(s0[c])));
+              s1[c] = __float_as_uint((c & 3) == 3 ? ex2_poly(__uint_as_float(s1[c])) : ex2(__uint_as_float(s1[c])));
+            }
+#pragma unroll
+            for (int c = 0; c < 16; ++c) {
+              pp[c] = pack_bf16(__uint_as_float(s0[2 * c]), __uint_as_float(s0[2 * c + 1]));
+              pp[16 + c] = pack_bf16(__uint_as_float(s1[2 * c]), __uint_as_float(s1[2 * c + 1]));
+            }
+          } else if (normal) {
+#pragma unroll
+            for (int c4 = 0; c4 < 8; ++c4) {
+#pragma unroll
+              for (int gg = 0; gg < 2; ++gg) {
+                uint32_t(&sv)[32] = gg ? s1 : s0;
+                const float4 l = lds_f4(m_ls + gg * 32 + 4 * c4), lo = lds_f4(m_lo + gg * 32 + 4 * c4), hi = lds_f4(m_hi + gg * 32 + 4 * c4);
+                const float lv[4] = {l.x, l.y, l.z, l.w};
+                const int lov[4] = {__float_as_int(lo.x), __float_as_int(lo.y), __float_as_int(lo.z), __float_as_int(lo.w)};
+                const int hiv[4] = {__float_as_int(hi.x), __float_as_int(hi.y), __float_as_int(hi.z), __float_as_int(hi.w)};
+#pragma unroll
+                for (int u = 0; u < 4; ++u) {
+                  const bool ok = kidx >= lov[u] && kidx < hiv[u];
+                  sv[4 * c4 + u] = ok ? __float_as_uint(fmaf(__uint_as_float(sv[4 * c4 + u]), SC, -lv[u])) : 0xff800000u;
+                }
+              }
+            }
+#pragma unroll
+            for (int c = 0; c < 32; ++c) {
+              s0[c] = __float_as_uint(ex2(__uint_as_float(s0[c])));
+              s1[c] = __float_as_uint(ex2(__uint_as_float(s1[c])));
+            }
+#pragma unroll
+            for (int c = 0; c < 16; ++c) {
+              pp[c] = pack_bf16(__uint_as_float(s0[2 * c]), __uint_as_float(s0[2 * c + 1]));
+              pp[16 + c] = pack_bf16(__uint_as_float(s1[2 * c]), __uint_as_float(s1[2 * c + 1]));
+            }
+          } else {
+#pragma unroll
+            for (int c = 0; c < 32; ++c) {
+              float e[2];
+#pragma unroll
+              for (int u = 0; u < 2; ++u) {
+                const int q = 2 * c + u;
+                const float rs = m_rs[q];
+                const bool ok = kidx >= m_lo[q] && kidx < m_hi[q];
+                const float sv = __uint_as_float(q < 32 ? s0[q & 31] : s1[q & 31]);
+                e[u] = ok ? ex2(fmaf(rs != 0.f ? sv : 0.f, rs, -m_ls[q])) : 0.f;
+              }
+              pp[c] = pack_bf16(e[0], e[1]);
+            }
+          }
+        }
+        if (warp == 0) TRACE(7, g);
+        tmem_st32(t_lane + cS + half * 64, pp);
+        uint32_t d0[32];
+        mbar_wait(dp_full, par);
         tc_fence_after();
-        if (warp == 0) TRACE(6, idx);
-        tmem_ld32(t_lane + cS + half * 64, s0);
-        tmem_ld32(t_lane + cS + half * 64 + 32, s1);
-        tmem_ld_wait();
+        if (g == gend - 1 && wait_tile(t + 1).n > 0) {
+          copy_next_kv();
+          cur |= 1;
+        }
+        tmem_ld32(t_lane + cDP + half * 64, d0);
+        tmem_st_wait();
         tc_fence_before();
         __syncwarp();
-        if (lane == 0) mbar_arrive(s_free);
-        if (inside) {
-#pragma unroll
-          for (int c4 = 0; c4 < 8; ++c4) {
-            const float4 la = lds_f4(m_ls + 4 * c4), lb = lds_f4(m_ls + 32 + 4 * c4);
-            s0[4 * c4] = __float_as_uint(fmaf(__uint_as_float(s0[4 * c4]), SC, -la.x));
-            s0[4 * c4 + 1] = __float_as_uint(fmaf(__uint_as_float(s0[4 * c4 + 1]), SC, -la.y));
-            s0[4 * c4 + 2] = __float_as_uint(fmaf(__uint_as_float(s0[4 * c4 + 2]), SC, -la.z));
-            s0[4 * c4 + 3] = __float_as_uint(fmaf(__uint_as_float(s0[4 * c4 + 3]), SC, -la.w));
-            s1[4 * c4] = __float_as_uint(fmaf(__uint_as_float(s1[4 * c4]), SC, -lb.x));
-            s1[4 * c4 + 1] = __float_as_uint(fmaf(__uint_as_float(s1[4 * c4 + 1]), SC, -lb.y));
-            s1[4 * c4 + 2] = __float_as_uint(fmaf(__uint_as_float(s1[4 * c4 + 2]), SC, -lb.z));
-            s1[4 * c4 + 3] = __float_as_uint(fmaf(__uint_as_float(s1[4 * c4 + 3]), SC, -lb.w));
-          }
-#pragma unroll
-          for (int c = 0; c < 32; ++c) {
-            s0[c] = __float_as_uint((c & 3) == 3 ? ex2_poly(__uint_as_float(s0[c])) : ex2(__uint_as_float(s0[c])));
-            s1[c] = __float_as_uint((c & 3) == 3 ? ex2_poly(__uint_as_float(s1[c])) : ex2(__uint_as_float(s1[c])));
-          }
-#pragma unroll
-          for (int c = 0; c < 16; ++c) {
-            pp[c] = pack_bf16(__uint_as_float(s0[2 * c]), __uint_as_float(s0[2 * c + 1]));
-            pp[16 + c] = pack_bf16(__uint_as_float(s1[2 * c]), __uint_as_float(s1[2 * c + 1]));
-          }
-        } else if (normal) {
-#pragma unroll
-          for (int c4 = 0; c4 < 8; ++c4) {
-#pragma unroll
-            for (int g = 0; g < 2; ++g) {
-              uint32_t(&sv)[32] = g ? s1 : s0;
-              const float4 l = lds_f4(m_ls + g * 32 + 4 * c4), lo = lds_f4(m_lo + g * 32 + 4 * c4), hi = lds_f4(m_hi + g * 32 + 4 * c4);
-              const float lv[4] = {l.x, l.y, l.z, l.w};
-              const int lov[4] = {__float_as_int(lo.x), __float_as_int(lo.y), __float_as_int(lo.z), __float_as_int(lo.w)};
-              const int hiv[4] = {__float_as_int(hi.x), __float_as_int(hi.y), __float_as_int(hi.z), __float_as_int(hi.w)};
-#pragma unroll
-              for (int u = 0; u < 4; ++u) {
-                const bool ok = kidx >= lov[u] && kidx < hiv[u];
-                sv[4 * c4 + u] = ok ? __float_as_uint(fmaf(__uint_as_float(sv[4 * c4 + u]), SC, -lv[u])) : 0xff800000u;
-              }
-            }
-          }
-#pragma unroll
-          for (int c = 0; c < 32; ++c) {
-            s0[c] = __float_as_uint(ex2(__uint_as_float(s0[c])));
-            s1[c] = __float_as_uint(ex2(__uint_as_float(s1[c])));
-          }
-#pragma unroll
-          for (int c = 0; c < 16; ++c) {
-            pp[c] = pack_bf16(__uint_as_float(s0[2 * c]), __uint_as_float(s0[2 * c + 1]));
-            pp[16 + c] = pack_bf16(__uint_as_float(s1[2 * c]), __uint_as_float(s1[2 * c + 1]));
-          }
-        } else {
-#pragma unroll
-          for (int c = 0; c < 32; ++c) {
-            float e[2];
-#pragma unroll
-            for (int u = 0; u < 2; ++u) {
-              const int q = 2 * c + u;
-              const float rs = m_rs[q];
-              const bool ok = kidx >= m_lo[q] && kidx < m_hi[q];
-              const float sv = __uint_as_float(q < 32 ? s0[q & 31] : s1[q & 31]);
-              e[u] = ok ? ex2(fmaf(rs != 0.f ? sv : 0.f, rs, -m_ls[q])) : 0.f;
-            }
-            pp[c] = pack_bf16(e[0], e[1]);
-          }
-        }
-      }
-      if (warp == 0) TRACE(7, idx);
-      tmem_st32(t_lane + cS + half * 64, pp);
-      uint32_t d0[32];
-      mbar_wait(dp_full, par);
-      tc_fence_after();
-      tmem_ld32(t_lane + cDP + half * 64, d0);
-      tmem_st_wait();
-      tc_fence_before();
-      __syncwarp();
-      if (lane == 0) mbar_arrive(p_full);
-      if (warp == 0) TRACE(8, idx);
-      auto dsmul = [&](const uint32_t (&d)[32], int hh) {
-        if (inside || normal) {
-#pragma unroll
-          for (int c4 = 0; c4 < 8; ++c4) {
-            const float4 nd = lds_f4(m_nd + hh * 32 + 4 * c4);
-            const uint32_t t0 = pack_bf16(fmaf(__uint_as_float(d[4 * c4]), RN, nd.x), fmaf(__uint_as_float(d[4 * c4 + 1]), RN, nd.y));
-            const uint32_t t1 = pack_bf16(fmaf(__uint_as_float(d[4 * c4 + 2]), RN, nd.z), fmaf(__uint_as_float(d[4 * c4 + 3]), RN, nd.w));
-            asm("mul.rn.bf16x2 %0, %1, %2;" : "=r"(pp[hh * 16 + 2 * c4]) : "r"(pp[hh * 16 + 2 * c4]), "r"(t0));
-            asm("mul.rn.bf16x2 %0, %1, %2;" : "=r"(pp[hh * 16 + 2 * c4 + 1]) : "r"(pp[hh * 16 + 2 * c4 + 1]), "r"(t1));
-          }
-        } else {
-#pragma unroll
-          for (int c4 = 0; c4 < 8; ++c4) {
-            const float4 nd = lds_f4(m_nd + hh * 32 + 4 * c4);
-            const float4 rs = lds_f4(m_rs + hh * 32 + 4 * c4);
-            const uint32_t t0 = pack_bf16(fmaf(__uint_as_float(d[4 * c4]), rs.x * kLn2, nd.x), fmaf(__uint_as_float(d[4 * c4 + 1]), rs.y * kLn2, nd.y));
-            const uint32_t t1 = pack_bf16(fmaf(__uint_as_float(d[4 * c4 + 2]), rs.z * kLn2, nd.z), fmaf(__uint_as_float(d[4 * c4 + 3]), rs.w * kLn2, nd.w));
-            asm("mul.rn.bf16x2 %0, %1, %2;" : "=r"(pp[hh * 16 + 2 * c4]) : "r"(pp[hh * 16 + 2 * c4]), "r"(t0));
-            asm("mul.rn.bf16x2 %0, %1, %2;" : "=r"(pp[hh * 16 + 2 * c4 + 1]) : "r"(pp[hh * 16 + 2 * c4 + 1]), "r"(t1));
-          }
-        }
-      };
-      tmem_ld_wait();
-      if (warp == 0) TRACE(9, idx);
-      dsmul(d0, 0);
-      if (warp == 0) TRACE(13, idx);
-      tmem_ld32(t_lane + cDP + half * 64 + 32, d0);
-      if (idx > 0) mbar_wait(ds_empty, (idx - 1) & 1);
-      tmem_ld_wait();
-      if (warp == 0) TRACE(14, idx);
-      dsmul(d0, 1);
-      if (warp == 0) TRACE(15, idx);
-      tmem_st32(t_lane + cDP + half * 64, pp);
-#pragma unroll
-      for (int c8 = 0; c8 < 8; ++c8)
-        *reinterpret_cast<uint4*>(pDS + swz_off(trow, c8)) = make_uint4(pp[4 * c8], pp[4 * c8 + 1], pp[4 * c8 + 2], pp[4 * c8 + 3]);
-      fence_async_smem();
-      tmem_st_wait();
-      tc_fence_before();
-      __syncwarp();
-      if (lane == 0) mbar_arrive(ds_full);
-      if (warp == 0) TRACE(10, idx);
+        if (lane == 0) mbar_arrive(p_full);
+        if (warp == 0) TRACE(8, g);
+        auto dsmul = [&](const uint32_t (&d)[32], int hh) {
+          if (inside || normal) {
+#pragma unroll
+            for (int c4 = 0; c4 < 8; ++c4) {
+              const float4 nd = lds_f4(m_nd + hh * 32 + 4 * c4);
+              const uint32_t t0 = pack_bf16(fmaf(__uint_as_float(d[4 * c4]), RN, nd.x), fmaf(__uint_as_float(d[4 * c4 + 1]), RN, nd.y));
+              const uint32_t t1 = pack_bf16(fmaf(__uint_as_float(d[4 * c4 + 2]), RN, nd.z), fmaf(__uint_as_float(d[4 * c4 + 3]), RN, nd.w));
+              asm("mul.rn.bf16x2 %0, %1, %2;" : "=r"(pp[hh * 16 + 2 * c4]) : "r"(pp[hh * 16 + 2 * c4]), "r"(t0));
+              asm("mul.rn.bf16x2 %0, %1, %2;" : "=r"(pp[hh * 16 + 2 * c4 + 1]) : "r"(pp[hh * 16 + 2 * c4 + 1]), "r"(t1));
+            }
+          } else {
+#pragma unroll
+            for (int c4 = 0; c4 < 8; ++c4) {
+              const float4 nd = lds_f4(m_nd + hh * 32 + 4 * c4);
+              const float4 rs = lds_f4(m_rs + hh * 32 + 4 * c4);
+              const uint32_t t0 = pack_bf16(fmaf(__uint_as_float(d[4 * c4]), rs.x * kLn2, nd.x), fmaf(__uint_as_float(d[4 * c4 + 1]), rs.y * kLn2, nd.y));
+              const uint32_t t1 = pack_bf16(fmaf(__uint_as_float(d[4 * c4 + 2]), rs.z * kLn2, nd.z), fmaf(__uint_as_float(d[4 * c4 + 3]), rs.w * kLn2, nd.w));
+              asm("mul.rn.bf16x2 %0, %1, %2;" : "=r"(pp[hh * 16 + 2 * c4]) : "r"(pp[hh * 16 + 2 * c4]), "r"(t0));
+              asm("mul.rn.bf16x2 %0, %1, %2;" : "=r"(pp[hh * 16 + 2 * c4 + 1]) : "r"(pp[hh * 16 + 2 * c4 + 1]), "r"(t1));
+            }
+          }
+        };
+        tmem_ld_wait();
+        if (warp == 0) TRACE(9, g);
+        dsmul(d0, 0);
+        if (warp == 0) TRACE(13, g);
+        tmem_ld32(t_lane + cDP + half * 64 + 32, d0);
+        if (g > 0) mbar_wait(ds_empty, (g - 1) & 1);
+        tmem_ld_wait();
+        if (warp == 0) TRACE(14, g);
+        dsmul(d0, 1);
+        if (warp == 0) TRACE(15, g);
+        tmem_st32(t_lane + cDP + half * 64, pp);
+#pragma unroll
+        for (int c8 = 0; c8 < 8; ++c8)
+          asm volatile("st.shared.v4.b32 [%0], {%1, %2, %3, %4};" ::"r"(aDS + swz_off(trow, c8)), "r"(pp[4 * c8]), "r"(pp[4 * c8 + 1]),
+                       "r"(pp[4 * c8 + 2]), "r"(pp[4 * c8 + 3]) : "memory");
+        fence_async_smem();
+        tmem_st_wait();
+        tc_fence_before();
+        __syncwarp();
+        if (lane == 0) mbar_arrive(ds_full);
+        if (warp == 0) TRACE(10, g);
+      }
+      release_tile(t);
     }
-    if (n > 0) {
-      mbar_wait(dkv_full, 0);
-      tc_fence_after();
-    }
-    if (warp == 0) TRACE(5, 61);
-#pragma unroll 1
-    for (int which = 0; which < 2; ++which) {
-      uint32_t v[32];
-      if (n > 0) {
-        tmem_ld32(t_lane + (which == 0 ? cDV : cDK) + half * 32, v);
-        tmem_ld_wait();
-      } else {
-#pragma unroll
-        for (int c = 0; c < 32; ++c) v[c] = 0u;
-      }
-      uint4 pk[4];
-#pragma unroll
-      for (int c8 = 0; c8 < 4; ++c8) {
-        pk[c8].x = pack_bf16(__uint_as_float(v[c8 * 8 + 0]), __uint_as_float(v[c8 * 8 + 1]));
-        pk[c8].y = pack_bf16(__uint_as_float(v[c8 * 8 + 2]), __uint_as_float(v[c8 * 8 + 3]));
-        pk[c8].z = pack_bf16(__uint_as_float(v[c8 * 8 + 4]), __uint_as_float(v[c8 * 8 + 5]));
-        pk[c8].w = pack_bf16(__uint_as_float(v[c8 * 8 + 6]), __uint_as_float(v[c8 * 8 + 7]));
-      }
-      if (p.tma_out) {
-        uint8_t* stage = which == 0 ? sQ : sDO;
-#pragma unroll
-        for (int c8 = 0; c8 < 4; ++c8) *reinterpret_cast<uint4*>(stage + swz_off(trow, half * 4 + c8)) = pk[c8];
-        if (warp == 0) TRACE(5, 52 - which);
-      } else if (kidx < p.Nk) {
-        uint16_t* out = (which == 0 ? p.dV + ((int64_t)b * p.Nk + kidx) * p.lddv : p.dK + ((int64_t)b * p.Nk + kidx) * p.lddk) +
-                        h * kD + half * 32;
-#pragma unroll
-        for (int c8 = 0; c8 < 4; ++c8) reinterpret_cast<uint4*>(out)[c8] = pk[c8];
-      }
-    }
-    if (p.tma_out) {
-      fence_async_smem();
-      asm volatile("bar.sync 1, 256;" ::: "memory");
-      if (warp == 0) TRACE(5, 50);
-      if (warp == 0 && lane == 0) {
-        tma_store_2d(&tmDV, sQ, h * kD, b * p.Nk + kv0);
-        tma_store_2d(&tmDK, sDO, h * kD, b * p.Nk + kv0);
-        tma_store_commit();
-        tma_store_wait_read();
-      }
-    }
-    if (warp == 0) TRACE(5, 60);
   }
   tc_fence_before();
   __syncthreads();
-  if (warp == 0) TRACE(5, 59);
+  if (warp == 0) TRACE_CTA(2);
   if (warp == kBwdMmaWarp) {
     tc_fence_after();
     tmem_dealloc<512>(tmem_base);
@@ -615,7 +730,10 @@
 
 #ifdef EGOM2P_TRACE
 extern "C" int egom2p_debug_attn_trace(long long* host_dst) {
-  return (int)cudaMemcpyFromSymbol(host_dst, egom2p::g_trace, sizeof(egom2p::g_trace));
+  cudaError_t e = cudaMemcpyFromSymbol(host_dst, egom2p::g_trace, sizeof(egom2p::g_trace));
+  if (e == cudaSuccess) e = cudaMemcpyFromSymbol(host_dst + 16 * 64, egom2p::g_trace_tile, sizeof(egom2p::g_trace_tile));
+  if (e == cudaSuccess) e = cudaMemcpyFromSymbol(host_dst + 16 * 64 + 64 * 4, egom2p::g_trace_cta, sizeof(egom2p::g_trace_cta));
+  return (int)e;
 }
 #endif
 
@@ -657,8 +775,8 @@
     if ((rc = make_tmap_2d(&tmDQ, dq_acc, 4, (uint64_t)B * Mq, (uint64_t)H * kD, (uint64_t)H * kD, 32, 32))) return rc;
     const int tma_out = (Nk % kT == 0 || B == 1) ? 1 : 0;
     if (tma_out) {
-      if ((rc = make_tmap_bf16_2d(&tmDK, dK, (uint64_t)B * Nk, (uint64_t)H * kD, lddk, kT, kD))) return rc;
-      if ((rc = make_tmap_bf16_2d(&tmDV, dV, (uint64_t)B * Nk, (uint64_t)H * kD, lddv, kT, kD))) return rc;
+      if ((rc = make_tmap_bf16_2d(&tmDK, dK, (uint64_t)B * Nk, (uint64_t)H * kD, lddk, 32, kD))) return rc;
+      if ((rc = make_tmap_bf16_2d(&tmDV, dV, (uint64_t)B * Nk, (uint64_t)H * kD, lddv, 32, kD))) return rc;
     } else {
       tmDK = tmK;
       tmDV = tmV;
diff --git a/egom2p_b200/csrc/common.cuh b/egom2p_b200/csrc/common.cuh
--- a/egom2p_b200/csrc/common.cuh
+++ b/egom2p_b200/csrc/common.cuh
@@ -153,6 +153,25 @@
   first_ctaid_x = (int)x;
   return valid != 0;
 }
+__device__ __forceinline__ void clc_try_cancel(void* resp16, uint64_t* bar) {
+  asm volatile("clusterlaunchcontrol.try_cancel.async.shared::cta.mbarrier::complete_tx::bytes.b128 [%0], [%1];"
+               ::"r"(smem_u32(resp16)), "r"(smem_u32(bar)) : "memory");
+}
+__device__ __forceinline__ bool clc_decode_xyz(const void* resp16, int& x, int& y, int& z) {
+  uint32_t valid, vx, vy, vz;
+  asm volatile(
+      "{\n\t.reg .pred p1;\n\t.reg .b128 r;\n\t"
+      "ld.shared.b128 r, [%4];\n\t"
+      "clusterlaunchcontrol.query_cancel.is_canceled.pred.b128 p1, r;\n\t"
+      "selp.u32 %3, 1, 0, p1;\n\t"
+      "mov.u32 %0, 0;\n\tmov.u32 %1, 0;\n\tmov.u32 %2, 0;\n\t"
+      "@p1 clusterlaunchcontrol.query_cancel.get_first_ctaid.v4.b32.b128 {%0, %1, %2, _}, r;\n\t}\n"
+      : "=r"(vx), "=r"(vy), "=r"(vz), "=r"(valid) : "r"(smem_u32(resp16)) : "memory");
+  x = (int)vx;
+  y = (int)vy;
+  z = (int)vz;
+  return valid != 0;
+}
 __device__ __forceinline__ uint32_t cluster_ctarank() {
   uint32_t r;
   asm volatile("mov.u32 %0, %%cluster_ctarank;" : "=r"(r));
```

After: 725,900, median of 6. 1.9% higher.
